# heracles-ec/heracles

Hardware: AMD Instinct MI355X
Metric: map->Cl pairs/sec + mixing-matrix build sec, nside=4096 lmax=6144 (higher is better)
Workload: dtype f64

## Files before the change

heracles_amd/_lib.py:

```python

from __future__ import annotations

import ctypes as C
import os
import threading

import numpy as np

_HERE = os.path.dirname(os.path.abspath(__file__))
_LIBNAME = os.environ.get("HX_LIBRARY") or os.path.join(_HERE, "libhxsht.so")
_lock = threading.Lock()
_lib = None

HX_OK = 0
HX_ERR_ARG, HX_ERR_NO_DEVICE, HX_ERR_HIP, HX_ERR_MEM, HX_ERR_UNSUPPORTED = -1, -2, -3, -4, -5

SYMBOLS = (
    "hx_version", "hx_last_error", "hx_device_count", "hx_init", "hx_set_stream",
    "hx_get_stream", "hx_set_async", "hx_synchronize", "hx_timer_start", "hx_timer_stop",
    "hx_profile_enable", "hx_profile_reset", "hx_profile_get", "hx_plan_create", "hx_set_max_lds_fft",
    "hx_plan_destroy", "hx_plan_scratch_bytes", "hx_plan_release_scratch", "hx_set_scratch_budget", "hx_plan_last_chunks", "hx_plan_mfma_flops", "hx_plan_executed_flops", "hx_executed_flops", "hx_measure_peaks", "hx_measured_mfma_clock", "hx_map2alm", "hx_map2alm_multi", "hx_map2alm_list", "hx_alm2map", "hx_copy",
    "hx_alm2cl_pairs", "hx_alm2cl_pairs_range", "hx_gauss_legendre", "hx_gauss_legendre_dd", "hx_wigner_d_table", "hx_mixmat",
    "hx_mixmat_eb", "hx_mixmat_eb_spin", "hx_mixmat_batch", "hx_mixctx_create", "hx_mixctx_apply", "hx_mixctx_apply_spin", "hx_mixctx_destroy", "hx_mixctx_set_bins", "hx_mixctx_apply_binned", "hx_mixctx_apply_binned_spin", "hx_cl2corr", "hx_corr2cl", "hx_cl2corr_cols", "hx_corr2cl_cols", "hx_cl2corr_cols_spin", "hx_corr2cl_cols_spin", "hx_xi_ratio", "hx_ang2pix_ring", "hx_map_values", "hx_ud_grade", "hx_reorder", "hx_matvec", "hx_pinv", "hx_alm_resample", "hx_region_maps", "hx_alm_subtract", "hx_fits_unpack_f64", "hx_fits_pack_f64", "hx_fits_unpack_columns",
    "hx_pointsht_create", "hx_pointsht_destroy", "hx_pointsht_info", "hx_pointsht_adjoint",
    "hx_pointsht_synthesis", "hx_pointsht_grids", "hx_pointgrid_gather", "hx_pointgrid_destroy",
    "hx_pixel_weights_size", "hx_pixel_weights_expand", "hx_pixel_weights_solve",
    "hx_ring_modes_size", "hx_ring_modes", "hx_legendre_from_modes", "hx_allgather_alms", "hx_host_alloc", "hx_host_free", "hx_mixmat_gemm_clock", "hx_mixmat_release", "hx_release_caches",
    "hx_cov_gram", "hx_cov_delete2", "hx_cov_shrink_sums",
    "hx_catmap_create", "hx_catmap_page", "hx_catmap_moments", "hx_catmap_finish", "hx_catmap_destroy",
    "hx_catalm_create", "hx_catalm_page", "hx_catalm_moments", "hx_catalm_finish", "hx_catalm_destroy",
    "hx_catmap_create_sel", "hx_catmap_page_sel", "hx_catmap_moments_sel", "hx_catmap_finish_sel", "hx_catmap_destroy_sel",
)


class HxError(RuntimeError):

    def __init__(self, code, msg):
        super().__init__(f"libhxsht error {code}: {msg}")
        self.code = code


def library_path() -> str:
    return _LIBNAME


def load():
    global _lib
    with _lock:
        if _lib is not None:
            return _lib
        if not os.path.exists(_LIBNAME):
            raise HxError(
                HX_ERR_NO_DEVICE,
                f"{_LIBNAME} not found: build it with `make -C heracles_amd/csrc` "
                "(hipcc, gfx950).  heracles_amd has no CPU fallback.",
            )
        try:
            import torch
        except ImportError:
            pass
        L = C.CDLL(_LIBNAME)
        vp, i, dp = C.c_void_p, C.c_int, C.c_void_p
        L.hx_version.restype = C.c_char_p
        L.hx_last_error.restype = C.c_char_p
        L.hx_get_stream.restype = vp
        L.hx_set_stream.argtypes = [vp]
        L.hx_plan_create.restype = vp
        L.hx_plan_create.argtypes = [i, i, i]
        L.hx_plan_destroy.argtypes = [vp]
        L.hx_plan_destroy.restype = None
        L.hx_plan_scratch_bytes.argtypes = [vp]
        L.hx_plan_scratch_bytes.restype = C.c_int64
        L.hx_plan_release_scratch.argtypes = [vp]
        L.hx_set_scratch_budget.argtypes = [C.c_double]
        L.hx_plan_last_chunks.argtypes = [vp]
        L.hx_plan_mfma_flops.argtypes = [vp, i, i, C.POINTER(C.c_double)]
        L.hx_plan_executed_flops.argtypes = [vp, i, i, C.POINTER(C.c_double)]
        L.hx_executed_flops.argtypes = [C.POINTER(C.c_double), i]
        L.hx_measure_peaks.argtypes = [C.POINTER(C.c_double)]
        L.hx_measured_mfma_clock.restype = C.c_double
        L.hx_map2alm.argtypes = [vp, i, i, dp, dp, dp, dp, dp, i]
        L.hx_alm2map.argtypes = [vp, i, i, dp, dp]
        L.hx_map2alm_multi.argtypes = [vp, i, vp, vp, vp, vp, dp, dp, vp]
        L.hx_map2alm_list.argtypes = [vp, i, vp, vp, vp, dp, dp, dp, dp, i]
        L.hx_copy.argtypes = [vp, vp, C.c_int64]
        L.hx_alm2cl_pairs.argtypes = [i, vp, vp, i, i, vp, vp, dp]
        L.hx_alm2cl_pairs_range.argtypes = [i, vp, vp, i, i, vp, vp, i, i, i, dp]
        L.hx_gauss_legendre.argtypes = [i, dp, dp]
        L.hx_gauss_legendre_dd.argtypes = [i, dp, dp, dp]
        L.hx_wigner_d_table.argtypes = [i, i, i, i, dp, dp]
        L.hx_mixmat.argtypes = [dp, i, i, i, i, i, i, dp]
        L.hx_mixmat_eb.argtypes = [dp, i, i, i, i, dp]
        L.hx_mixmat_eb_spin.argtypes = [dp, i, i, i, i, i, i, dp]
        L.hx_mixmat_batch.argtypes = [i, dp, i, i, i, i, vp, vp, vp, vp]
        L.hx_mixctx_create.restype = vp
        L.hx_mixctx_create.argtypes = [i, i, i]
        L.hx_mixctx_apply.argtypes = [vp, dp, i, i, dp]
        L.hx_mixctx_destroy.argtypes = [vp]
        L.hx_mixctx_set_bins.argtypes = [vp, i, vp, dp, dp]
        L.hx_mixctx_apply_binned.argtypes = [vp, dp, i, i, dp]
        L.hx_mixctx_apply_spin.argtypes = [vp, dp, i, i, i, dp]
        L.hx_mixctx_apply_binned_spin.argtypes = [vp, dp, i, i, i, dp]
        L.hx_mixctx_destroy.restype = None
        L.hx_cl2corr.argtypes = [i, i, dp, dp]
        L.hx_corr2cl.argtypes = [i, i, dp, dp]
        L.hx_cl2corr_cols.argtypes = [i, i, i, vp, dp, dp]
        L.hx_corr2cl_cols.argtypes = [i, i, i, vp, dp, dp]
        L.hx_cl2corr_cols_spin.argtypes = [i, i, i, vp, dp, dp]
        L.hx_corr2cl_cols_spin.argtypes = [i, i, i, vp, dp, dp]
        L.hx_xi_ratio.argtypes = [i, i, dp, dp, vp, dp, vp, vp, C.c_double, C.c_double, dp]
        L.hx_ang2pix_ring.argtypes = [i, C.c_int64, dp, dp, dp]
        L.hx_map_values.argtypes = [i, C.c_int64, dp, dp, i, dp, dp, i]
        L.hx_ud_grade.argtypes = [i, i, i, dp, dp]
        L.hx_reorder.argtypes = [i, i, i, dp, dp]
        L.hx_matvec.argtypes = [i, i, dp, i, dp, dp]
        L.hx_pinv.argtypes = [i, i, dp, C.c_double, dp, C.POINTER(C.c_double)]
        L.hx_alm_resample.argtypes = [i, i, i, dp, dp]
        L.hx_region_maps.argtypes = [C.c_int64, i, dp, dp, C.c_double, dp]
        L.hx_alm_subtract.argtypes = [C.c_int64, dp, i, vp, dp]
        L.hx_fits_unpack_f64.argtypes = [C.c_int64, i, i, C.c_int64, C.c_int64, C.c_int64, dp, dp]
        L.hx_fits_pack_f64.argtypes = [C.c_int64, i, i, C.c_int64, C.c_int64, C.c_int64, dp, dp]
        L.hx_fits_unpack_columns.argtypes = [C.c_int64, C.c_int64, i, vp, C.c_char_p, vp, vp, dp, vp, i]
        L.hx_pointsht_create.argtypes = [i, C.c_double]
        L.hx_pointsht_create.restype = vp
        L.hx_pointsht_destroy.argtypes = [vp]
        L.hx_pointsht_destroy.restype = None
        L.hx_pointsht_info.argtypes = [vp, C.POINTER(C.c_int)]
        L.hx_pointsht_adjoint.argtypes = [vp, i, i, C.c_int64, dp, dp, dp]
        L.hx_pointsht_synthesis.argtypes = [vp, i, i, C.c_int64, dp, dp, dp]
        L.hx_pointsht_grids.argtypes = [vp, i, i, dp]
        L.hx_pointsht_grids.restype = vp
        L.hx_pointgrid_gather.argtypes = [vp, C.c_int64, dp, dp]
        L.hx_pointgrid_destroy.argtypes = [vp]
        L.hx_pointgrid_destroy.restype = None
        L.hx_ring_modes_size.argtypes = [vp, i]
        L.hx_ring_modes_size.restype = C.c_int64
        L.hx_ring_modes.argtypes = [vp, i, dp, dp, dp, i, vp, vp, i, vp]
        L.hx_legendre_from_modes.argtypes = [vp, i, i, vp, i, i, i, dp, dp]
        L.hx_allgather_alms.argtypes = [vp, i, vp, dp]
        L.hx_pixel_weights_size.argtypes = [i]
        L.hx_pixel_weights_size.restype = C.c_int64
        L.hx_pixel_weights_expand.argtypes = [i, C.c_int64, dp, dp]
        L.hx_pixel_weights_solve.argtypes = [vp, i, C.c_double, i, dp, C.POINTER(C.c_int), C.POINTER(C.c_double), C.POINTER(C.c_double)]
        L.hx_host_alloc.argtypes = [C.c_int64, C.POINTER(C.c_void_p)]
        L.hx_host_free.argtypes = [vp]
        L.hx_mixmat_gemm_clock.restype = C.c_double
        L.hx_timer_stop.argtypes = [C.POINTER(C.c_float)]
        L.hx_cov_gram.argtypes = [i, i, i, dp, dp, C.c_double, dp]
        L.hx_cov_delete2.argtypes = [i, i, i, dp, dp, dp, vp, vp, i, vp, C.c_double, dp]
        L.hx_cov_shrink_sums.argtypes = [i, i, dp, dp, C.c_int64, dp]
        L.hx_catmap_create.restype = vp
        L.hx_catmap_create.argtypes = [C.c_int64, i, i, vp, vp]
        L.hx_catmap_page.argtypes = [vp, C.c_int64, vp]
        L.hx_catmap_moments.argtypes = [vp, dp, dp]
        L.hx_catmap_finish.argtypes = [vp, i, C.c_double, dp]
        L.hx_catmap_destroy.argtypes = [vp]
        L.hx_catmap_destroy.restype = None
        L.hx_catalm_create.restype = vp
        L.hx_catalm_create.argtypes = [C.c_int64, i, i, vp, vp]
        L.hx_catalm_page.argtypes = [vp, C.c_int64, vp]
        L.hx_catalm_moments.argtypes = [vp, dp, dp]
        L.hx_catalm_finish.argtypes = [vp, i, i, C.c_double, dp, dp]
        L.hx_catalm_destroy.argtypes = [vp]
        L.hx_catalm_destroy.restype = None
        L.hx_catmap_create_sel.restype = vp
        L.hx_catmap_create_sel.argtypes = [C.c_int64, i, i, vp, i, i, vp, vp, i, vp, vp, vp]
        L.hx_catmap_page_sel.argtypes = [vp, C.c_int64, vp, vp]
        L.hx_catmap_moments_sel.argtypes = [vp, dp, dp, dp]
        L.hx_catmap_finish_sel.argtypes = [vp, i, i, C.c_double, dp]
        L.hx_catmap_destroy_sel.argtypes = [vp]
        L.hx_catmap_destroy_sel.restype = None
        L.hx_profile_get.argtypes = [C.c_char_p, C.POINTER(C.c_int), C.POINTER(C.c_double)]
        _lib = L
        return L


def check(rc: int):
    if rc != HX_OK:
        raise HxError(rc, load().hx_last_error().decode(errors="replace"))


def ptr(obj):
    if obj is None:
        return None
    if isinstance(obj, int):
        return C.c_void_p(obj)
    if isinstance(obj, np.ndarray):
        if not obj.flags.c_contiguous:
            raise ValueError("array must be C-contiguous")
        return C.c_void_p(obj.ctypes.data)
    if hasattr(obj, "data_ptr"):
        if not obj.is_contiguous():
            raise ValueError("tensor must be contiguous")
        if getattr(obj, "is_cuda", False):
            import torch

            torch.cuda.current_stream(obj.device).synchronize()
        return C.c_void_p(obj.data_ptr())
    raise TypeError(f"cannot take the address of {type(obj)!r}")


def init(device: int | None = None):
    L = load()
    if device is None:
        device = int(os.environ.get("LOCAL_RANK", "0")) % max(L.hx_device_count(), 1)
    check(L.hx_init(int(device)))
    global _inited, _device
    _inited, _device = True, int(device)


_inited = False
_device = None


def ensure_init():
    global _inited
    if not _inited:
        init(None)
        _inited = True


def device() -> int:
    ensure_init()
    return _device


def device_count() -> int:
    return load().hx_device_count()


def measure_peaks():
    ensure_init()
    out = (C.c_double * 4)()
    check(load().hx_measure_peaks(out))
    return {"hbm_read_gbs": out[0], "hbm_copy_gbs": out[1], "fp64_mfma_tflops": out[2], "fp64_valu_tflops": out[3],
            "fp64_mfma_clock_ghz": load().hx_measured_mfma_clock()}


def synchronize():
    check(load().hx_synchronize())


def release_caches():
    from . import weights

    weights.release_computed()
    check(load().hx_release_caches())


def copy(dst, src):
    nb = int(src.nbytes) if hasattr(src, "nbytes") else int(src.numel() * src.element_size())
    nd = int(dst.nbytes) if hasattr(dst, "nbytes") else int(dst.numel() * dst.element_size())
    if nb != nd:
        raise ValueError(f"copy of {nb} bytes into {nd}")
    check(load().hx_copy(ptr(dst), ptr(src), nb))


def executed_flops(reset=False):
    ensure_init()
    out = (C.c_double * 2)()
    check(load().hx_executed_flops(out, 1 if reset else 0))
    return out[0], out[1]


def set_scratch_budget(nbytes: float):
    check(load().hx_set_scratch_budget(float(nbytes)))


class Timer:

    def __enter__(self):
        check(load().hx_timer_start())
        self.ms = None
        return self

    def __exit__(self, *exc):
        t = C.c_float()
        check(load().hx_timer_stop(C.byref(t)))
        self.ms = float(t.value)
        return False


def profile_enable(on=True):
    check(load().hx_profile_enable(1 if on else 0))


def profile_reset():
    check(load().hx_profile_reset())


def profile_get(name: str):
    n = C.c_int()
    ms = C.c_double()
    check(load().hx_profile_get(name.encode(), C.byref(n), C.byref(ms)))
    return n.value, ms.value


def pinned_empty(shape, dtype=None):
    import weakref

    dtype = np.dtype(np.float64 if dtype is None else dtype)
    shape = tuple(int(x) for x in (shape if isinstance(shape, (tuple, list)) else (shape,)))
    nbytes = int(np.prod(shape, dtype=np.int64)) * dtype.itemsize
    if nbytes == 0:
        return np.empty(shape, dtype)
    ensure_init()
    L = load()
    p = C.c_void_p()
    check(L.hx_host_alloc(C.c_int64(nbytes), C.byref(p)))
    raw = (C.c_char * nbytes).from_address(p.value)
    weakref.finalize(raw, L.hx_host_free, C.c_void_p(p.value))
    return np.frombuffer(raw, dtype=dtype).reshape(shape)


def result_array(shape, out=None):
    shape = tuple(int(x) for x in shape)
    if out is None:
        return np.empty(shape)
    if tuple(out.shape) != shape:
        raise ValueError(f"out has shape {tuple(out.shape)}, the result has {shape}")
    if isinstance(out, np.ndarray):
        if out.dtype != np.float64 or not out.flags.c_contiguous or not out.flags.writeable:
            raise ValueError("out must be a writeable C-contiguous float64 array")
    elif hasattr(out, "data_ptr"):
        import torch

        if out.dtype != torch.float64 or not out.is_contiguous():
            raise ValueError("out must be a contiguous float64 tensor")
    else:
        raise TypeError(f"out: cannot write into {type(out)!r}")
    return out
```

heracles_amd/csrc/hx_analysis.hip:

```cpp
#include <algorithm>
#include <cmath>
#include <cstdlib>
#include <cstring>

#include "hx_sht_common.h"

namespace hx {
using namespace hxfft;

constexpr int HALF_F = 1;
template <int SPIN>
struct LegCfg {
    static constexpr int NW = SPIN == 0 ? 16 : 8;
    static constexpr int NT = SPIN == 0 ? 1 : 2;
    static constexpr int NOP = SPIN == 0 ? 1 : 2;
    static constexpr int NPAR = (SPIN == 2 && HALF_F) ? 1 : 2;
};
int analysis_f_rows(int spin) { return spin == 0 ? LegCfg<0>::NPAR * LegCfg<0>::NOP : LegCfg<2>::NPAR * LegCfg<2>::NOP; }

struct LegParams {
    PlanDev P;
    const LegTask *__restrict__ tasks;
    const double *__restrict__ F;
    double *__restrict__ partial;
    int m0, ms;
    long long row0;
    int ng;
    int ncol;
    int pcol;
    const MTasks *__restrict__ of_m;
    const long long *__restrict__ arow;
    long long arow0;
    int add_all;
};

constexpr int COMB_NXCD = 8, COMB_XG = 4;
constexpr int COMB_TM = 16;
constexpr int COMB_IPT = 3;
constexpr int COMB_MPAD = 2;
static int combine_rp(int rowlen) { return rowlen <= 40 ? 8 : 4; }
static size_t combine_lds_bytes(int rp, int rowlen)
{
    return (size_t)COMB_TM * ((size_t)rp * rowlen + COMB_MPAD) * sizeof(double) + (size_t)COMB_TM * rp * sizeof(RingAtM) + COMB_TM * sizeof(int);
}
template <int SPIN, int RP>
__global__ __launch_bounds__(1024) void k_fourier_combine(PlanDev P, const double2 *__restrict__ Y, int ncomp, int ncol, int m0, int ms,
                                                         int nm, int kshift, int gx, int gy, const double *__restrict__ rw,
                                                         const LegTask *__restrict__ tasks, const MTasks *__restrict__ of_m,
                                                         double *__restrict__ F, int tile0)
{
    constexpr int NOP = LegCfg<SPIN>::NOP, NPAR = LegCfg<SPIN>::NPAR, TM = COMB_TM;
    const int bq = (int)blockIdx.x / (COMB_NXCD * COMB_XG), br = (int)blockIdx.x % (COMB_NXCD * COMB_XG);
    const int t = (bq * COMB_NXCD + br % COMB_NXCD) * COMB_XG + br / COMB_NXCD;
    if (t >= gx * gy) return;
    const int tx = t % gx, ty = t / gx;
    static_assert(TM == 16 && 32 % RP == 0 && TM * RP <= 256, "tile shape");
    extern __shared__ __align__(16) unsigned char comb_lds[];
    const int rowlen = NPAR * NOP * ncol;
    const int mstride = RP * rowlen + COMB_MPAD;
    double *tile = reinterpret_cast<double *>(comb_lds);
    RingAtM *ring_at_m = reinterpret_cast<RingAtM *>(tile + TM * mstride);
    int *m_live = reinterpret_cast<int *>(ring_at_m + TM * RP);
    const int kb = tx * TM - kshift;
    const int rp0 = (ty + tile0 * (32 / RP)) * RP;
    if (threadIdx.x < TM * RP) {
        const int mi = threadIdx.x % TM, j = threadIdx.x / TM, k = kb + mi;
        bool on = k >= 0 && k < nm;
        if (on) {
            const int m = m0 + k * ms;
            const MTasks mt = of_m[m];
            on = mt.count != 0 && rp0 / 32 >= tasks[mt.first].rb0;
            if (on) ring_at_m[j * TM + mi] = ring_at_m_of(P, rp0 + j, m, rw);
        }
        if (j == 0) m_live[mi] = on;
    }
    __syncthreads();
    const int nsl = ncol >> 1;
    for (int e = threadIdx.x; e < RP * nsl * TM; e += blockDim.x) {
        const int i = e % TM, sj = e / TM, s = sj % nsl, j = sj / nsl;
        const int mi = ((i & 3) << 2) | (i >> 2);
        if (!m_live[mi]) continue;
        const int m = m0 + (kb + mi) * ms, rp = rp0 + j;
        const bool live = rp < P.nrp;
        const RingAtM ram = ring_at_m[j * TM + mi];
        double *row = tile + mi * mstride + j * rowlen;
        if (SPIN == 0) {
            const int c = s;
            double2 sm = make_double2(0.0, 0.0), d = sm;
            if (live && c < ncomp) {
                double2 fn, fs;
                ring_modes_ns(P, Y, c, rp, m, ram, fn, fs);
                sm = cadd(fn, fs);
                d = csub(fn, fs);
            }
            *reinterpret_cast<double2 *>(row + 2 * s) = sm;
            *reinterpret_cast<double2 *>(row + ncol + 2 * s) = d;
        } else {
            const int f = s >> 1, op = s & 1;
            double4 o0 = make_double4(0.0, 0.0, 0.0, 0.0), o1 = o0;
            if (live && 2 * f + 1 < ncomp) {
                double2 qn, qs, un, us;
                ring_modes_ns(P, Y, 2 * f, rp, m, ram, qn, qs);
                ring_modes_ns(P, Y, 2 * f + 1, rp, m, ram, un, us);
                const double2 ppn = cscale(cadd(qn, mul_pi(un)), -0.5), pmn = cscale(csub(qn, mul_pi(un)), -0.5);
                const double2 pps = cscale(cadd(qs, mul_pi(us)), -0.5), pms = cscale(csub(qs, mul_pi(us)), -0.5);
                double4 x, y;
                if (op == 0) {
                    x = make_double4(ppn.x, ppn.y, ppn.y, -ppn.x);
                    y = make_double4(pms.x, pms.y, -pms.y, pms.x);
                } else {
                    x = make_double4(pmn.x, pmn.y, -pmn.y, pmn.x);
                    y = make_double4(pps.x, pps.y, pps.y, -pps.x);
                }
                o0 = make_double4(x.x + y.x, x.y + y.y, x.z + y.z, x.w + y.w);
                o1 = make_double4(x.x - y.x, x.y - y.y, x.z - y.z, x.w - y.w);
            }
            double2 *t0 = reinterpret_cast<double2 *>(row + (0 * NOP + op) * ncol + 4 * f);
            t0[0] = make_double2(o0.x, o0.y);
            t0[1] = make_double2(o0.z, o0.w);
            if (NPAR == 2) {
                double2 *t1 = reinterpret_cast<double2 *>(row + (1 * NOP + op) * ncol + 4 * f);
                t1[0] = make_double2(o1.x, o1.y);
                t1[1] = make_double2(o1.z, o1.w);
            }
        }
    }
    __syncthreads();
    const int lane = threadIdx.x & 63, npiece = RP * rowlen / 2, cpm = (npiece + 63) / 64;
    for (int ch = threadIdx.x >> 6; ch < TM * cpm; ch += blockDim.x >> 6) {
        const int mi = ch / cpm, u = (ch % cpm) * 64 + lane;
        if (!m_live[mi] || u >= npiece) continue;
        const double2 *src = reinterpret_cast<const double2 *>(tile + mi * mstride);
        double2 *dst = reinterpret_cast<double2 *>(F + ((long long)(kb + mi) * P.nrp_pad + rp0) * rowlen);
        dst[u] = src[u];
    }
}

template <int SPIN>
static void launch_fourier_combine(hipStream_t st, const PlanDev &P, const double2 *Y, int ncomp, int ncol, int m0, int ms, int nm, const double *d_rw,
                                   const LegTask *tasks, const MTasks *of_m, double *F, int tile0, int ntile32)
{
    const int kshift = ms == 1 ? m0 % COMB_TM : 0;
    const int rowlen = LegCfg<SPIN>::NPAR * LegCfg<SPIN>::NOP * ncol;
    const int gx = (nm + kshift + COMB_TM - 1) / COMB_TM;
    static_assert((size_t)COMB_TM * (4 * LegCfg<SPIN>::NPAR * LegCfg<SPIN>::NOP * (NCOL * NGMAX + 8) + COMB_MPAD) * sizeof(double) +
                          (size_t)COMB_TM * 4 * sizeof(RingAtM) + COMB_TM * sizeof(int) <= 65536, "a tile of 4 ring pairs must fit 64 KiB of LDS");
    const int rp = combine_rp(rowlen), items = rp * (ncol / 2) * COMB_TM;
    const unsigned nt = (unsigned)std::min(1024, std::max(COMB_TM * rp, (items / COMB_IPT + 63) / 64 * 64));
    const int gy = ntile32 * (32 / rp);
    const dim3 grid((unsigned)((gx * gy + COMB_NXCD * COMB_XG - 1) / (COMB_NXCD * COMB_XG) * (COMB_NXCD * COMB_XG)));
    const size_t lds = combine_lds_bytes(rp, rowlen);
    if (rp == 8)
        hipLaunchKernelGGL((k_fourier_combine<SPIN, 8>), grid, dim3(nt), lds, st, P, Y, ncomp, ncol, m0, ms, nm, kshift, gx, gy, d_rw, tasks, of_m, F, tile0);
    else
        hipLaunchKernelGGL((k_fourier_combine<SPIN, 4>), grid, dim3(nt), lds, st, P, Y, ncomp, ncol, m0, ms, nm, kshift, gx, gy, d_rw, tasks, of_m, F, tile0);
}

__device__ __host__ inline int tile_swz(int r) { return r & 15; }
__device__ __host__ inline int ringsel(int q, int k) { return (k & 1) * 16 + 2 * q + (k >> 1); }

template <int K>
__device__ inline int opaque(int v)
{
    asm("; opaque %1" : "+v"(v) : "n"(K));
    return v;
}

__device__ unsigned long long g_exec_flops[2];

template <int SPIN>
struct PipeCfg {
    static constexpr int NW = 4;
    static constexpr int RBS = SPIN == 0 ? 2 : 1;
    static constexpr int NCH = SPIN == 0 ? 2 : 1;
    static constexpr int NOP = SPIN == 0 ? 1 : 2;
};

__device__ __host__ inline int pipe_rho(int q, int k) { return 4 * q + k; }
__device__ __host__ inline int pipe_tile_idx(int c, int r) { return c * 32 + ((r ^ (c & 7)) * 2); }

constexpr int DUO_GAP = -1;
constexpr int DUO_PRIO = 1;
constexpr int DUO_ORDER = -1;
constexpr int DUO_SCALE_BITS2 = 100;
constexpr int DUO_SCALE_BITS0 = 300;

template <int K>
__device__ __forceinline__ double row_bcast(double v)
{
    double d;
    asm("v_mov_b64_dpp %0, %1 row_newbcast:%2 row_mask:0xf bank_mask:0xf" : "=v"(d) : "v"(v), "n"(K));
    return d;
}

template <int K>
__device__ __forceinline__ double row_bcast_fmac(double t, double p, double x)
{
    asm("v_fmac_f64_dpp %0, %1, %2 row_newbcast:%3 row_mask:0xf bank_mask:0xf" : "+v"(t) : "v"(p), "v"(x), "n"(K));
    return t;
}

template <int SPIN>
__device__ __forceinline__ void alm_rows_to_layout(const PlanDev &P, int m, bool any_task, const double *__restrict__ partial, long long r0, int ncol,
                                                   int ncomp, int ng, const double *__restrict__ fl, int add, double2 *__restrict__ alm,
                                                   long long alm_stride, const double *__restrict__ alphan, int tid, int nt)
{
    const int lmax = P.lmax;
    const int l0 = SPIN == 0 ? m : (m > 2 ? m : 2);
    const int nl = lmax - m + 1, nc = 8 * ng;
    constexpr int U = 8;
    for (int i0 = tid; i0 < nl * nc; i0 += nt * U) {
        double2 v[U];
        double al[U], f[U];
        long long dsti[U];
        bool on[U];
#pragma unroll
        for (int u = 0; u < U; ++u) {
            const int i = i0 + u * nt;
            const int l = m + i / nc, c = i % nc;
            on[u] = i < nl * nc && c < ncomp;
            v[u] = make_double2(0.0, 0.0);
            al[u] = 1.0;
            f[u] = 1.0;
            dsti[u] = 0;
            if (!on[u]) continue;
            dsti[u] = (long long)c * alm_stride + almidx(lmax, l, m);
            if (l >= l0 && any_task) {
                const double *prow = partial + (r0 + (l - l0)) * ncol + (c >> 3) * NCOL;
                v[u] = *reinterpret_cast<const double2 *>(prow + 2 * (c & 7));
                if (SPIN == 2 && alphan && ((l + m) & 1)) {
                    const int j = 2 * (c & 7);
                    v[u] = make_double2(prow[j ^ 3], prow[(j + 1) ^ 3]);
                }
                if (SPIN == 2 && HALF_F && ((l + m) & 1)) {
                    if (c & 1) v[u].y = -v[u].y;
                    else v[u].x = -v[u].x;
                }
                if (alphan) al[u] = alphan[almidx(lmax, l, m)];
                if (fl) f[u] = fl[l];
            }
        }
#pragma unroll
        for (int u = 0; u < U; ++u) {
            if (!on[u]) continue;
            double2 w = v[u];
            if (alphan) { w.x *= al[u]; w.y *= al[u]; }
            if (fl) { w.x *= f[u]; w.y *= f[u]; }
            double2 *dst = alm + dsti[u];
            if (add) { const double2 o = *dst; w.x += o.x; w.y += o.y; }
            *dst = w;
        }
    }
}

template <int SPIN, int NG, int NBX, int NSUB = 1>
__global__ __launch_bounds__(256, 2) void k_legendre_duo(LegParams A, const double2 *__restrict__ coefn)
{
    using C = PipeCfg<SPIN>;
    constexpr int NW = 4, NOP = C::NOP, NCH = C::NCH, NPAIR = 16;
    constexpr int NXA = NBX > 0 ? NBX : 1;
    constexpr int DQ0 = NG * 512, DSZ = NG * 512 + NBX * 128;
    constexpr bool HALFB = SPIN == 2;
    constexpr int SB = SPIN == 2 ? DUO_SCALE_BITS2 : DUO_SCALE_BITS0;
    constexpr int GAPN = DUO_GAP >= 0 ? DUO_GAP : ((SPIN == 2 && NG == 2 && NBX == 2) ? 5 : (SPIN == 2 && NG == 2 && NBX == 1) ? 6 : (SPIN == 2 && NG == 1 && NBX == 2) ? 0 : 4);
    constexpr int GORDER = DUO_ORDER >= 0 ? DUO_ORDER : ((SPIN == 2 && NG == 2 && NBX == 2) ? 2 : (SPIN == 0 && NG == 1 && NBX == 1) ? 1 : 0);
    constexpr int NPB = HALFB ? 1 : 2;
    constexpr int TW = NSUB * DSZ > 2048 ? NSUB * DSZ : 2048;
    static_assert(NG >= 1 && NG <= 2 && TW * NW * 8 <= 81920, "two work-groups per CU");
    static_assert(SPIN == 0 || HALF_F, "spin 2: the lambda- chain carries (-1)^(l + m) lambda- (one operand row, wave-uniform coefficients)");
    __shared__ double tile[NW][TW];
    __shared__ int lead_in[2][NW];
    const PlanDev &P = A.P;
    const int m = A.m0 + blockIdx.x * A.ms, lmax = P.lmax;
    const MTasks mt = A.of_m[m];
    const int l0 = SPIN == 0 ? m : (m > 2 ? m : 2);
    const int off = (l0 + m) & 1;
    const int nblk = (lmax - l0) / LBLK + 1;
    const long long orow = A.arow[m] - A.arow0;
    const double2 *__restrict__ cfm = coefn + almidx(lmax, 0, m) + l0 + (SPIN == 0 ? 0 : 1) + (threadIdx.x & 15);
    bool first_group = true;
    auto put = [&](double *p, double v) __attribute__((always_inline)) {
        if (first_group) *p = v;
        else __builtin_amdgcn_global_atomic_fadd_f64((__attribute__((address_space(1))) double *)p, v);
    };
    auto lds_barrier = []() __attribute__((always_inline)) {
        __builtin_amdgcn_s_waitcnt(0xc07f);
        __builtin_amdgcn_s_barrier();
    };
    int n_mf = 0, n_rec = 0;
    if (DUO_PRIO) __builtin_amdgcn_s_setprio(3);
    for (int ti = 0; ti < mt.count; ++ti) {
        const LegTask task = A.tasks[mt.first + ti];
        first_group = ti == 0 && !A.add_all;
        int tid = threadIdx.x;
        asm volatile("; ring group" : "+v"(tid));
        const int w = tid >> 6, lane = tid & 63;
        const int ai = lane & 15, ak = lane >> 4;
        if (ti) __syncthreads();

        const int rbi = SPIN == 0 ? 2 * w + (lane >> 5) : w;
        const int rpl = (task.rb0 + rbi) * RBLK + (lane & 31);
        const bool valid = rbi < task.nrb && rpl < P.nrp;
        const double x = valid ? P.z[rpl] : 0.0;
        const double xx = SPIN == 0 ? x * x : ((lane >> 5) ? -x : x);

        double fr[NPAIR][NPB][NG], frx[NPAIR][NPB][NXA];
#pragma unroll
        for (int sp = 0; sp < NPAIR; ++sp) {
            const int op = SPIN == 0 ? 0 : sp & 1, q = SPIN == 0 ? sp : sp >> 1;
            const int rbq = SPIN == 0 ? 2 * w + (q >> 3) : w;
            const bool on = rbq < task.nrb;
            const long long row = (long long)blockIdx.x * P.nrp_pad + (task.rb0 + rbq) * RBLK + pipe_rho(q & 7, ak);
            if (HALFB) {
                const double *f = A.F + (row * NOP + op) * A.ncol;
#pragma unroll
                for (int g = 0; g < NG; ++g) fr[sp][0][g] = on ? f[g * NCOL + ai] : 0.0;
#pragma unroll
                for (int g = 0; g < NXA; ++g) frx[sp][0][g] = (NBX > 0 && on) ? f[NG * NCOL + 4 * g + (lane & 3)] : 0.0;
            } else {
#pragma unroll
                for (int pos = 0; pos < NPB; ++pos) {
                    const double *f = A.F + ((row * 2 + (pos ^ off)) * NOP + op) * A.ncol;
#pragma unroll
                    for (int g = 0; g < NG; ++g) fr[sp][pos][g] = on ? f[g * NCOL + ai] : 0.0;
#pragma unroll
                    for (int g = 0; g < NXA; ++g) frx[sp][pos][g] = (NBX > 0 && on) ? f[NG * NCOL + 4 * g + (lane & 3)] : 0.0;
                }
            }
        }

        double vc[NCH], vp[NCH];
        int sc[NCH];
#pragma unroll
        for (int c = 0; c < NCH; ++c) { vc[c] = 0.0; vp[c] = 0.0; sc[c] = -100; }
        if (valid) {
            if (SPIN == 0) {
                SVal a = spow(P.sth[rpl], m);
                a.v *= P.mfac[m];
                SVal b = a;
                b.v *= sqrt(2.0 * m + 3.0) * P.z[rpl];
                snorm_small(a);
                snorm_small(b);
                vc[0] = a.v; sc[0] = a.e;
                vc[NCH - 1] = b.v; sc[NCH - 1] = b.e;
            } else {
                SVal sp, sm;
                spin2_seeds(m, P.sth[rpl], P.omz[rpl], P.kfac2[m], sp, sm);
                vc[0] = (lane >> 5) ? (off ? -sm.v : sm.v) : sp.v;
                sc[0] = (lane >> 5) ? sm.e : sp.e;
            }
#pragma unroll
            for (int c = 0; c < NCH; ++c) sval_rebase<SB>(vc[c], sc[c]);
        }

        auto rec_step = [&](auto RMM, int c, int step, const double tq) __attribute__((always_inline)) {
            constexpr int RM = decltype(RMM)::value;
            if (RM != 3 && (step & 3) == 0) {
                const int hc = __double2hiint(vc[c]), hp = __double2hiint(vp[c]);
                const bool up = sc[c] < 0 && (hc & 0x7ff00000) >= 0x3ff00000;
                const int sub = up ? (SB << 20) : 0;
                const bool pz = up && (hp & 0x7ff00000) <= (SB << 20);
                vc[c] = __hiloint2double(hc - sub, __double2loint(vc[c]));
                vp[c] = pz ? 0.0 : __hiloint2double(hp - sub, __double2loint(vp[c]));
                sc[c] += up ? 1 : 0;
            }
            const double cur = (RM == 3 || sc[c] == 0) ? vc[c] : 0.0;
            const double vn = fma(tq, vc[c], -vp[c]);
            vp[c] = vc[c];
            vc[c] = vn;
            return cur;
        };
        constexpr int HB = 8;
        double *tw = &tile[w][0];
        auto recursion = [&](auto RMM, const double2 (&cl)[2]) __attribute__((always_inline)) {
            constexpr int RM = decltype(RMM)::value;
#pragma unroll
            for (int h = 0; h < LBLK / HB; ++h) {
                double cur[HB];
#pragma unroll
                for (int k = 0; k < HB; ++k) {
                    constexpr int dummy = 0; (void)dummy;
                    const int kk = HB * h + k;
                    double tq = 0.0;
                    switch (kk & 15) {
#define HX_BC(K) case K: tq = row_bcast_fmac<K>(row_bcast<K>(cl[kk >> 4].y), cl[kk >> 4].x, xx); break;
                        HX_BC(0) HX_BC(1) HX_BC(2) HX_BC(3) HX_BC(4) HX_BC(5) HX_BC(6) HX_BC(7)
                        HX_BC(8) HX_BC(9) HX_BC(10) HX_BC(11) HX_BC(12) HX_BC(13) HX_BC(14) HX_BC(15)
#undef HX_BC
                    }
                    cur[k] = rec_step(RMM, SPIN == 0 ? ((kk & 1) ? NCH - 1 : 0) : 0, SPIN == 0 ? kk >> 1 : kk, tq);
                }
                if (RM >= 2) {
#pragma unroll
                    for (int j = 0; j < HB / 2; ++j)
                        *reinterpret_cast<double2 *>(tw + pipe_tile_idx(lane, h * (HB / 2) + j)) = make_double2(cur[2 * j], cur[2 * j + 1]);
                }
                __builtin_amdgcn_sched_barrier(0);
            }
        };
        auto set_mode = [&](int b) __attribute__((always_inline)) {
            const int eb = b == 0 ? 60 : (b == 1 ? 34 : (30 - 2 * b > 8 ? 30 - 2 * b : 8));
            auto lane_dead = [&](int c) __attribute__((always_inline)) {
                if (SB == 300) return sc[c] < 0;
                const int ef = (__double2hiint(vc[c]) >> 20) & 0x7ff;
                return sc[c] <= -2 || (sc[c] == -1 && ef <= 1022 - eb);
            };
            bool dead = !valid || lane_dead(0), live = !valid || sc[0] == 0;
            if (NCH == 2) {
                dead = dead && (!valid || lane_dead(NCH - 1));
                live = live && (!valid || sc[NCH - 1] == 0);
            }
            return __all(dead) ? 1 : (__all(live) ? 3 : 2);
        };
        using I1 = std::integral_constant<int, 1>;
        using I2 = std::integral_constant<int, 2>;
        using I3 = std::integral_constant<int, 3>;

        const int fcol = tid & 15, fch = (tid >> 4) & 7, fpos = (tid >> 7) & 1;
        const int frow = (fch >> 1) + 8 * (fch & 1);
        const int qrow = tid / (4 * NXA), qcol = tid % (4 * NXA);
        double *pgrp = A.partial + (orow + 2 * frow + fpos) * A.pcol + fcol;
        double *pquad = A.partial + (orow + 2 * qrow) * A.pcol + NG * NCOL + qcol;
        double2 cnext[2] = {cfm[0], cfm[16]};
        bool started = first_group;
        int nflush = 0;
        for (int b0 = 0; b0 < nblk; b0 += NSUB) {
            double4_t acc[NSUB][NG][2];
            double accx[NSUB][NXA][2];
            bool mine = false;
#pragma unroll
            for (int sub = 0; sub < NSUB; ++sub) {
                const int b = b0 + sub;
#pragma unroll
                for (int g = 0; g < NG; ++g) acc[sub][g][0] = acc[sub][g][1] = (double4_t){0.0, 0.0, 0.0, 0.0};
#pragma unroll
                for (int g = 0; g < NXA; ++g) accx[sub][g][0] = accx[sub][g][1] = 0.0;
                if (b >= nblk) break;
                int rm = set_mode(b);
                const double2 cl[2] = {cnext[0], cnext[1]};
                if (rm == 3) recursion(I3{}, cl);
                else if (rm == 2) {
                    recursion(I2{}, cl);
                    if (SB != 300) {
                        bool lv = valid && sc[0] == 0;
                        if (NCH == 2) lv = lv || (valid && sc[NCH - 1] == 0);
                        if (!__any(lv)) rm = 1;
                    }
                } else recursion(I1{}, cl);
                cnext[0] = cfm[(b + 1) * LBLK];
                cnext[1] = cfm[(b + 1) * LBLK + 16];
                n_rec = __builtin_amdgcn_readfirstlane(n_rec + 1);
                mine = mine || rm >= 2;
                if (rm >= 2) {
                    n_mf = __builtin_amdgcn_readfirstlane(n_mf + 1);
                    if (DUO_PRIO) __builtin_amdgcn_s_setprio(0);
                    constexpr int PF = 3;
                    auto a_fetch = [&](int sp) __attribute__((always_inline)) {
                        const int op = SPIN == 0 ? 0 : sp & 1, q = SPIN == 0 ? sp : sp >> 1;
                        const int c = SPIN == 0 ? (q >> 3) * 32 + pipe_rho(q & 7, ak) : op * 32 + pipe_rho(q, ak);
                        return *reinterpret_cast<const double2 *>(tw + pipe_tile_idx(c, ai));
                    };
                    double2 aq[PF + 1];
#pragma unroll
                    for (int j = 0; j < PF; ++j) aq[j] = a_fetch(j);
#pragma unroll
                    for (int sp = 0; sp < NPAIR; ++sp) {
                        if (sp + PF < NPAIR) aq[(sp + PF) % (PF + 1)] = a_fetch(sp + PF);
                        const double a0 = aq[sp % (PF + 1)].x, a1 = aq[sp % (PF + 1)].y;
#pragma unroll
                        for (int pos = 0; pos < 2; ++pos) {
                            const double a = pos ? a1 : a0;
                            if (GAPN > 0) {
                                if (GORDER == 1) {
#pragma unroll
                                for (int g = 0; g < (NG > NBX ? NG : NBX); ++g) {
                                    if (g < NG) acc[sub][g][pos] = __builtin_amdgcn_mfma_f64_16x16x4f64(a, fr[sp][HALFB ? 0 : pos][g], acc[sub][g][pos], 0, 0, 0);
                                    __builtin_amdgcn_sched_barrier(0);
                                    asm volatile("s_nop %0" ::"n"(GAPN > 0 ? GAPN - 1 : 0));
                                    __builtin_amdgcn_sched_barrier(0);
                                    if (g < NBX) accx[sub][g][pos] = __builtin_amdgcn_mfma_f64_4x4x4f64(a, frx[sp][HALFB ? 0 : pos][g], accx[sub][g][pos], 0, 0, 0);
                                    __builtin_amdgcn_sched_barrier(0);
                                }
                                } else if (GORDER == 2) {
#pragma unroll
                                for (int g = 0; g < NG; ++g) acc[sub][g][pos] = __builtin_amdgcn_mfma_f64_16x16x4f64(a, fr[sp][HALFB ? 0 : pos][g], acc[sub][g][pos], 0, 0, 0);
                                __builtin_amdgcn_sched_barrier(0);
                                asm volatile("s_nop %0" ::"n"(GAPN > 0 ? GAPN - 1 : 0));
                                __builtin_amdgcn_sched_barrier(0);
#pragma unroll
                                for (int g = 0; g < NBX; ++g) accx[sub][g][pos] = __builtin_amdgcn_mfma_f64_4x4x4f64(a, frx[sp][HALFB ? 0 : pos][g], accx[sub][g][pos], 0, 0, 0);
                                __builtin_amdgcn_sched_barrier(0);
                                if (NBX > 0) asm volatile("s_nop %0" ::"n"(GAPN > 0 ? GAPN - 1 : 0));
                                __builtin_amdgcn_sched_barrier(0);
                                } else {
#pragma unroll
                                for (int g = 0; g < (NG > NBX ? NG : NBX); ++g) {
                                    if (g < NG) acc[sub][g][pos] = __builtin_amdgcn_mfma_f64_16x16x4f64(a, fr[sp][HALFB ? 0 : pos][g], acc[sub][g][pos], 0, 0, 0);
                                    if (g < NBX) accx[sub][g][pos] = __builtin_amdgcn_mfma_f64_4x4x4f64(a, frx[sp][HALFB ? 0 : pos][g], accx[sub][g][pos], 0, 0, 0);
                                    __builtin_amdgcn_sched_barrier(0);
                                    asm volatile("s_nop %0" ::"n"(GAPN > 0 ? GAPN - 1 : 0));
                                    __builtin_amdgcn_sched_barrier(0);
                                }
                                }
                            } else {
#pragma unroll
                                for (int g = 0; g < NG; ++g) acc[sub][g][pos] = __builtin_amdgcn_mfma_f64_16x16x4f64(a, fr[sp][HALFB ? 0 : pos][g], acc[sub][g][pos], 0, 0, 0);
#pragma unroll
                                for (int g = 0; g < NBX; ++g) accx[sub][g][pos] = __builtin_amdgcn_mfma_f64_4x4x4f64(a, frx[sp][HALFB ? 0 : pos][g], accx[sub][g][pos], 0, 0, 0);
                            }
                        }
                        __builtin_amdgcn_sched_barrier(0);
                    }
                    if (DUO_PRIO) __builtin_amdgcn_s_setprio(3);
                }
            }
            const bool two = NSUB > 1 && b0 + 1 < nblk;
            if (!started) {
                if (lane == 0) lead_in[nflush & 1][w] = mine ? 1 : 0;
                lds_barrier();
                const int4 fl = *reinterpret_cast<const int4 *>(&lead_in[nflush & 1][0]);
                ++nflush;
                started = __builtin_amdgcn_readfirstlane(fl.x | fl.y | fl.z | fl.w) != 0;
                if (!started) {
                    pgrp += (long long)NSUB * LBLK * A.pcol;
                    pquad += (long long)NSUB * LBLK * A.pcol;
                    continue;
                }
            }
#pragma unroll
            for (int sub = 0; sub < NSUB; ++sub) {
                double *dt = tw + sub * DSZ;
#pragma unroll
                for (int g = 0; g < NG; ++g)
#pragma unroll
                    for (int pos = 0; pos < 2; ++pos)
#pragma unroll
                        for (int h = 0; h < 2; ++h)
                            *reinterpret_cast<double2 *>(dt + (g * 2 + pos) * 256 + ai * 16 + (((2 * ak + h) ^ (ai & 7)) * 2)) = make_double2(acc[sub][g][pos][2 * h], acc[sub][g][pos][2 * h + 1]);
#pragma unroll
                for (int g = 0; g < NBX; ++g)
                    *reinterpret_cast<double2 *>(dt + DQ0 + ((4 * ((lane >> 2) & 3) + ak) * 4 * NBX + 4 * g + (lane & 3)) * 2) = make_double2(accx[sub][g][0], accx[sub][g][1]);
            }
            lds_barrier();
#pragma unroll
            for (int sub = 0; sub < NSUB; ++sub) {
                if (sub > 0 && !two) break;
                const long long rsub = (long long)sub * LBLK * A.pcol;
#pragma unroll
                for (int g = 0; g < NG; ++g) {
                    const double *src = &tile[0][0] + sub * DSZ + (g * 2 + fpos) * 256 + fcol * 16 + ((fch ^ (fcol & 7)) * 2);
                    double2 s4[NW];
#pragma unroll
                    for (int ww = 0; ww < NW; ++ww) s4[ww] = *reinterpret_cast<const double2 *>(src + ww * TW);
                    put(pgrp + rsub + g * NCOL, (s4[0].x + s4[1].x) + (s4[2].x + s4[3].x));
                    put(pgrp + rsub + g * NCOL + 8 * (long long)A.pcol, (s4[0].y + s4[1].y) + (s4[2].y + s4[3].y));
                }
                if (NBX > 0 && tid < 64 * NBX) {
                    double2 s4[NW];
#pragma unroll
                    for (int ww = 0; ww < NW; ++ww) s4[ww] = *reinterpret_cast<const double2 *>(&tile[0][0] + ww * TW + sub * DSZ + DQ0 + tid * 2);
                    put(pquad + rsub, (s4[0].x + s4[1].x) + (s4[2].x + s4[3].x));
                    put(pquad + rsub + A.pcol, (s4[0].y + s4[1].y) + (s4[2].y + s4[3].y));
                }
            }
            pgrp += (long long)NSUB * LBLK * A.pcol;
            pquad += (long long)NSUB * LBLK * A.pcol;
            lds_barrier();
        }
    }
    if ((threadIdx.x & 63) == 0) {
        atomicAdd(&g_exec_flops[0], (unsigned long long)n_mf * (32ull * (NG * 2048ull + NBX * 512ull)));
        atomicAdd(&g_exec_flops[1], (unsigned long long)n_rec * (64ull * LBLK * 4ull));
    }
}

template <int SPIN>
__global__ __launch_bounds__(256) void k_alm_reduce(PlanDev P, const LegTask *__restrict__ tasks,
                                                    const MTasks *__restrict__ of_m,
                                                    const double *__restrict__ partial, long long row0, int m0, int ms,
                                                    int ncomp, int ng, int ncol, const double *__restrict__ fl, int add,
                                                    double2 *__restrict__ alm, long long alm_stride,
                                                    const long long *__restrict__ arow, const double *__restrict__ alphan)
{
    const int m = m0 + blockIdx.x * ms, lmax = P.lmax;
    const int l0 = SPIN == 0 ? m : (m > 2 ? m : 2);
    const MTasks mt = of_m[m];
    const int nl = lmax - m + 1, nc = 8 * ng;
    if (arow) {
        alm_rows_to_layout<SPIN>(P, m, mt.count > 0, partial, arow[m] - row0, ncol, ncomp, ng, fl, add, alm, alm_stride, alphan, threadIdx.x, blockDim.x);
        return;
    }
    for (int i = threadIdx.x; i < nl * nc; i += blockDim.x) {
        const int l = m + i / nc, c = i % nc;
        if (c >= ncomp) continue;
        double2 v = make_double2(0.0, 0.0);
        if (l >= l0) {
            const int col = (c >> 3) * NCOL + 2 * (c & 7);
            for (int t = 0; t < mt.count; ++t) {
                const double *p = partial + (tasks[mt.first + t].pout - row0 + (l - l0)) * ncol + col;
                v.x += p[0];
                v.y += p[1];
            }
            if (fl) { v.x *= fl[l]; v.y *= fl[l]; }
        }
        double2 *dst = alm + (long long)c * alm_stride + almidx(lmax, l, m);
        if (add) { const double2 o = *dst; v.x += o.x; v.y += o.y; }
        *dst = v;
    }
}

__global__ __launch_bounds__(256) void k_alm_reduce_spin(int lmax, int s, const LegTask *__restrict__ tasks, const MTasks *__restrict__ of_m,
                                                         const double *__restrict__ partial, long long row0, int m0, int ms,
                                                         const double *__restrict__ fl, int add, double2 *__restrict__ alm, long long alm_stride)
{
    const int m = m0 + blockIdx.x * ms;
    const int l0 = m > s ? m : s;
    const MTasks mt = of_m[m];
    const int nl = lmax - m + 1;
    for (int i = threadIdx.x; i < nl * 2; i += blockDim.x) {
        const int l = m + (i >> 1), c = i & 1;
        double2 v = make_double2(0.0, 0.0);
        if (l >= l0) {
            for (int t = 0; t < mt.count; ++t) {
                const double *p = partial + (tasks[mt.first + t].pout - row0 + (l - l0)) * 4 + 2 * c;
                v.x += p[0];
                v.y += p[1];
            }
            if (fl) { v.x *= fl[l]; v.y *= fl[l]; }
        }
        double2 *dst = alm + (long long)c * alm_stride + almidx(lmax, l, m);
        if (add) { const double2 o = *dst; v.x += o.x; v.y += o.y; }
        *dst = v;
    }
}

struct SweepShape {
    int ng, nbx, valu, ncol, duo;
};
static SweepShape sweep_shape(int spin, int nb)
{
    const int cols = 2 * nb;
    SweepShape sh = {0, 0, 0, 0, 0};
    if (cols <= 8) { sh.valu = 1; return sh; }
    sh.duo = 1;
    sh.ng = std::max(cols / NCOL, 1);
    const int rem = cols > NCOL ? cols % NCOL : 0;
    const int maxbx = spin == 2 ? 2 : (sh.ng == 1 ? 1 : 0);
    if (rem > 4 * maxbx) sh.ng += 1;
    else sh.nbx = (rem + 3) / 4;
    sh.ncol = NCOL * sh.ng + 4 * sh.nbx;
    return sh;
}
bool analysis_generic_spin(int spin)
{
    if (spin != 2) return spin != 0;
    const char *e = getenv("HX_SPIN_GENERIC");
    return e && atoi(e) != 0;
}
int analysis_max_comp(int spin) { return spin == 2 ? 8 * NGMAX + 4 : 8 * NGMAX; }

static double sweep_cost(int spin, int units)
{
    if (spin == 0) return units <= 4 ? 21.6 * units : (units <= 8 ? 84.1 : (units <= 10 ? 99.2 : 139.7));
    return units <= 2 ? 61.0 * units : (units <= 4 ? 164.5 : (units == 5 ? 194.1 : (units == 6 ? 222.0 : (units <= 8 ? 272.0 : (units == 9 ? 299.6 : 326.0)))));
}
int analysis_next_batch(int spin, int remaining)
{
    const int unit = spin == 0 ? 1 : 2, maxu = analysis_max_comp(spin) / unit;
    const int units = remaining / unit;
    if (units <= 0) return 0;
    std::vector<double> best(units + 1, 0.0);
    std::vector<int> first(units + 1, 0);
    for (int r = 1; r <= units; ++r) {
        best[r] = 1e300;
        for (int b = std::min(maxu, r); b >= 1; --b) {
            const double c = sweep_cost(spin, b) + best[r - b];
            if (c < best[r] - 1e-9) { best[r] = c; first[r] = b; }
        }
    }
    return unit * first[units];
}
int analysis_max_batch(int spin, int ncomp)
{
    int mx = 0;
    for (int left = ncomp; left > 0;) {
        const int nb = analysis_next_batch(spin, left);
        if (nb <= 0) break;
        mx = std::max(mx, nb);
        left -= nb;
    }
    return mx;
}

int one_set_task_blocks(int spin) { return PipeCfg<2>::NW * (spin ? PipeCfg<2>::RBS : PipeCfg<0>::RBS); }
int flop_task_blocks(int spin) { return spin == 0 ? LegCfg<0>::NW : LegCfg<2>::NW; }

static bool duo_shape(const SweepShape &sh) { return sh.duo != 0; }
static int sweep_pcol(const SweepShape &sh) { return sh.ncol > 2 * NCOL ? (sh.ncol + 15) / 16 * 16 : sh.ncol; }

template <int SPIN>
static int launch_duo(const SweepShape &sh, dim3 pgrid, hipStream_t st, const LegParams &A, const double2 *cn)
{
    const dim3 db(256);
    const int key = sh.ng * 10 + sh.nbx;
    if (key == 10) hipLaunchKernelGGL((k_legendre_duo<SPIN, 1, 0, 2>), pgrid, db, 0, st, A, cn);
    else if (key == 11) hipLaunchKernelGGL((k_legendre_duo<SPIN, 1, 1, 2>), pgrid, db, 0, st, A, cn);
    else if (key == 20 && SPIN == 2) hipLaunchKernelGGL((k_legendre_duo<2, 2, 0, 2>), pgrid, db, 0, st, A, cn);
    else if (key == 12 && SPIN == 2) hipLaunchKernelGGL((k_legendre_duo<2, 1, 2, 2>), pgrid, db, 0, st, A, cn);
    else if (key == 21 && SPIN == 2) hipLaunchKernelGGL((k_legendre_duo<2, 2, 1, 2>), pgrid, db, 0, st, A, cn);
    else if (key == 20) hipLaunchKernelGGL((k_legendre_duo<SPIN, 2, 0>), pgrid, db, 0, st, A, cn);
    else if (key == 22 && SPIN == 2) hipLaunchKernelGGL((k_legendre_duo<2, 2, 2>), pgrid, db, 0, st, A, cn);
    else return fail(HX_ERR_ARG, "legendre analysis: no two-group kernel for %d groups + %d blocks", sh.ng, sh.nbx);
    return HX_OK;
}

static void launch_alm_reduce(hx_plan *pl, int spin, hx_plan::TaskSet &ts, long long row0, int m0, int ms, int nm, int nb, int ng, int pcol,
                              const double *d_fl, int add, double2 *d_alms, const double *al)
{
    const PlanDev P = pl->dev();
    const long long *arow = al ? ts.d_arow.as<long long>() : nullptr;
    if (spin == 0)
        hipLaunchKernelGGL(k_alm_reduce<0>, dim3(nm), dim3(256), 0, rt().stream, P, ts.d_tasks.as<LegTask>(), ts.d_of_m.as<MTasks>(), pl->partial.as<double>(),
                           row0, m0, ms, nb, ng, pcol, d_fl, add, d_alms, pl->nlm, arow, al);
    else
        hipLaunchKernelGGL(k_alm_reduce<2>, dim3(nm), dim3(256), 0, rt().stream, P, ts.d_tasks.as<LegTask>(), ts.d_of_m.as<MTasks>(), pl->partial.as<double>(),
                           row0, m0, ms, nb, ng, pcol, d_fl, add, d_alms, pl->nlm, arow, al);
}

template <int SPIN>
static int launch_chunk(hx_plan *pl, hx_plan::SpinData &sd, hx_plan::TaskSet &ts, int m0, int m1, int nb, const SweepShape &sh, const double *d_rw,
                        const double *d_fl, int add, double2 *d_alms)
{
    const int ng = sh.ng + (sh.nbx > 0 ? 1 : 0), ncol = sh.ncol;
    const int pcol = sweep_pcol(sh);
    hipStream_t st = rt().stream;
    PlanDev P = pl->dev();
    const int t0 = ts.of_m[m0].first;
    const int t1 = ts.of_m[m1 - 1].first + ts.of_m[m1 - 1].count;
    const int ms = std::max(pl->m_step, 1), nm = (m1 - m0 + ms - 1) / ms;
    {
        ProfScope ps("fourier_combine");
        launch_fourier_combine<SPIN>(st, P, pl->Y.as<double2>(), nb, ncol, m0, ms, nm, d_rw, ts.d_tasks.as<LegTask>(), ts.d_of_m.as<MTasks>(),
                                     pl->F.as<double>(), 0, pl->nrp_pad / 32);
    }
    if (t1 > t0) {
        ProfScope ps("legendre_analysis");
        ProfScope ps2(SPIN == 0 ? "legendre_analysis_s0" : "legendre_analysis_s2");
        LegParams A;
        A.P = P; A.tasks = ts.d_tasks.as<LegTask>() + t0; A.F = pl->F.as<double>(); A.partial = pl->partial.as<double>();
        A.m0 = m0; A.ms = ms; A.row0 = ts.rows_before_m[m0]; A.ng = ng; A.ncol = ncol; A.pcol = pcol;
        A.of_m = ts.d_of_m.as<MTasks>(); A.arow = ts.d_arow.as<long long>(); A.arow0 = ts.arow[m0]; A.add_all = 0;
        A.tasks = ts.d_tasks.as<LegTask>();
        HX_TRY(launch_duo<SPIN>(sh, dim3((unsigned)nm), st, A, sd.cn.as<double2>()));
    }
    {
        ProfScope ps("alm_reduce");
        launch_alm_reduce(pl, SPIN, ts, ts.arow[m0], m0, ms, nm, nb, ng, pcol, d_fl, add, d_alms, sd.al.as<double>());
    }
    HX_HIP(hipGetLastError());
    return HX_OK;
}

static bool valu_batch(int spin, int nb) { return sweep_shape(spin, nb).valu != 0; }

static double analysis_budget(const hx_plan *pl)
{
    if (scratch_budget_bytes() > 0.0) return scratch_budget_bytes();
    double budget = 80e9;
    size_t fr = 0, tot = 0;
    if (hipMemGetInfo(&fr, &tot) == hipSuccess) budget = std::min(budget, 0.5 * (double)(fr + pl->F.bytes + pl->partial.bytes));
    return std::max(budget, 2e9);
}

static int plan_m_chunks(hx_plan *pl, double f_per_m, const std::vector<long long> &prow, size_t row_bytes, std::vector<std::pair<int, int>> &chunks)
{
    const double budget = analysis_budget(pl);
    size_t maxF = 16, maxP = 16;
    const int m_end = pl->m_hi < 0 ? pl->lmax + 1 : std::min(pl->m_hi, pl->lmax + 1), ms = std::max(pl->m_step, 1);
    for (int m0 = std::max(pl->m_lo, 0); m0 < m_end;) {
        int last = m0;
        while (last + ms < m_end) {
            const double bytes = f_per_m * ((last + ms - m0) / ms + 1) + (double)(prow[last + ms + 1] - prow[m0]) * row_bytes;
            if (bytes > budget) break;
            last += ms;
        }
        const int m1 = last + 1;
        chunks.emplace_back(m0, m1);
        maxF = std::max(maxF, (size_t)(f_per_m * ((m1 - m0 + ms - 1) / ms)));
        maxP = std::max(maxP, (size_t)(prow[m1] - prow[m0]) * row_bytes);
        m0 = last + ms;
    }
    HX_TRY(pl->F.alloc(maxF));
    HX_TRY(pl->partial.alloc(maxP));
    pl->last_chunks = (int)chunks.size();
    return HX_OK;
}

static int analysis_batch_valu(hx_plan *pl, int spin, int nb, const double *d_maps, double2 *d_alms, const double *d_rw,
                               const double *d_pw, const double *d_fl, int add, bool generic = false)
{
    hx_plan::SpinData *sd = nullptr;
    hx_plan::TaskSet *tsp = nullptr;
    HX_TRY(spin_data(pl, spin, generic, &sd));
    HX_TRY(task_set(pl, spin, generic, valu_task_blocks(spin), &tsp));
    hx_plan::TaskSet &ts = *tsp;
    if (pl->hsrc == nullptr && pl->nssrc == nullptr) {
        HX_TRY(pl->Y.alloc(sizeof(double2) * (size_t)pl->ny * nb));
        HX_TRY(launch_ring_subdft_maps(pl, nb, d_maps, d_pw, pl->Y.as<double2>()));
    }
    const int lmax = pl->lmax, pcol = valu_partial_cols(spin), unit = spin ? 2 : 1, ms = std::max(pl->m_step, 1);
    std::vector<std::pair<int, int>> chunks;
    HX_TRY(plan_m_chunks(pl, (double)pl->nrp_pad * valu_operand_doubles(spin) * sizeof(double), ts.rows_before_m, pcol * sizeof(double), chunks));
    for (int c0 = 0; c0 < nb; c0 += unit)
        for (auto &ch : chunks) {
            const int m0 = ch.first, m1 = ch.second, nm = (m1 - m0 + ms - 1) / ms;
            HX_TRY(launch_valu_chunk(pl, spin, *sd, ts, m0, m1, c0, d_rw, generic));
            ProfScope ps("alm_reduce");
            if (generic)
                hipLaunchKernelGGL(k_alm_reduce_spin, dim3(nm), dim3(256), 0, rt().stream, lmax, spin, ts.d_tasks.as<LegTask>(), ts.d_of_m.as<MTasks>(),
                                   pl->partial.as<double>(), ts.rows_before_m[m0], m0, ms, d_fl, add, d_alms + (size_t)c0 * pl->nlm, pl->nlm);
            else
                launch_alm_reduce(pl, spin, ts, ts.rows_before_m[m0], m0, ms, nm, unit, 1, pcol, d_fl, add, d_alms + (size_t)c0 * pl->nlm, nullptr);
            HX_HIP(hipGetLastError());
        }
    return HX_OK;
}

int analysis_batch(hx_plan *pl, int spin, int nb, const double *d_maps, double2 *d_alms, const double *d_rw,
                   const double *d_pw, const double *d_fl, int add)
{
    const bool generic = plan_generic_spin(pl, spin);
    if (generic || (spin != 0 && spin != 2)) {
        if (!generic) return fail(HX_ERR_UNSUPPORTED, "spin-%d maps not yet supported", spin);
        if (spin < 0 || nb < 2 || (nb & 1)) return fail(HX_ERR_ARG, "analysis_batch: %d components of spin %d", nb, spin);
        if (spin > pl->lmax) {
            if (!add) HX_HIP(hipMemsetAsync(d_alms, 0, sizeof(double2) * (size_t)pl->nlm * nb, rt().stream));
            return HX_OK;
        }
        return analysis_batch_valu(pl, spin, nb, d_maps, d_alms, d_rw, d_pw, d_fl, add, true);
    }
    if (valu_batch(spin, nb)) return analysis_batch_valu(pl, spin, nb, d_maps, d_alms, d_rw, d_pw, d_fl, add);
    const SweepShape sh = sweep_shape(spin, nb);
    hx_plan::TaskSet *ts = nullptr;
    hx_plan::SpinData *sd = nullptr;
    HX_TRY(spin_data(pl, spin, false, &sd));
    HX_TRY(task_set(pl, spin, false, one_set_task_blocks(spin), &ts));
    if (pl->hsrc == nullptr && pl->nssrc == nullptr) {
        HX_TRY(pl->Y.alloc(sizeof(double2) * (size_t)pl->ny * nb));
        HX_TRY(launch_ring_subdft_maps(pl, nb, d_maps, d_pw, pl->Y.as<double2>()));
    }
    std::vector<std::pair<int, int>> chunks;
    HX_TRY(plan_m_chunks(pl, (double)pl->nrp_pad * analysis_f_rows(spin) * sh.ncol * sizeof(double), ts->arow, sweep_pcol(sh) * sizeof(double), chunks));
    for (auto &ch : chunks) {
        if (spin == 0)
            HX_TRY(launch_chunk<0>(pl, *sd, *ts, ch.first, ch.second, nb, sh, d_rw, d_fl, add, d_alms));
        else
            HX_TRY(launch_chunk<2>(pl, *sd, *ts, ch.first, ch.second, nb, sh, d_rw, d_fl, add, d_alms));
    }
    return HX_OK;
}

bool analysis_can_stream(hx_plan *pl, int spin, int nb)
{
    if (!pl || pl->nside < 1 || pl->hsrc || pl->nssrc || pl->m_lo != 0 || pl->m_hi >= 0 || pl->m_step > 1) return false;
    if (nb < 1 || nb > analysis_max_comp(spin)) return false;
    const SweepShape sh = sweep_shape(spin, nb);
    if (!duo_shape(sh) || sh.valu) return false;
    const double f_bytes = (double)pl->nrp_pad * analysis_f_rows(spin) * sh.ncol * sizeof(double) * (pl->lmax + 1.0);
    const double p_bytes = 0.5 * (pl->lmax + 1.0) * (pl->lmax + 2.0 + LBLK) * sweep_pcol(sh) * sizeof(double);
    double budget = 80e9;
    if (scratch_budget_bytes() > 0.0) budget = scratch_budget_bytes();
    if (f_bytes + p_bytes > budget) return false;
    size_t fr = 0, tot = 0;
    if (hipMemGetInfo(&fr, &tot) != hipSuccess) {
        (void)hipGetLastError();
        return false;
    }
    const double y_bytes = (double)pl->ny * nb * sizeof(double2), stage_bytes = 2.0 * nb * (double)pl->npix * sizeof(double);
    const double held = (double)pl->F.bytes + (double)pl->partial.bytes + (double)pl->Y.bytes + (double)pl->stage[0].bytes + (double)pl->stage[1].bytes +
                        (double)pl->stage[2].bytes;
    return f_bytes + p_bytes + y_bytes + stage_bytes <= 0.95 * ((double)fr + held);
}

int analysis_stream_plan(hx_plan *pl, int spin, int nb, int nslab, StreamSweep &s)
{
    if (!analysis_can_stream(pl, spin, nb)) return fail(HX_ERR_ARG, "analysis_stream_plan: not a streamable sweep");
    HX_TRY(spin_data(pl, spin, false, &s.sd));
    HX_TRY(task_set(pl, spin, false, one_set_task_blocks(spin), &s.ts));
    hx_plan::TaskSet &ts = *s.ts;
    const SweepShape sh = sweep_shape(spin, nb);
    s.pl = pl; s.spin = spin; s.nb = nb;
    const int nrb = (pl->nrp + RBLK - 1) / RBLK;
    std::vector<double> cum(nrb + 1, 0.0);
    for (int rb = 0; rb < nrb; ++rb) {
        double px = 0.0;
        for (int rp = rb * RBLK; rp < std::min((rb + 1) * RBLK, pl->nrp); ++rp) px += (rp == pl->nrp - 1 ? 4.0 : 8.0) * pl->h_nsub[rp];
        cum[rb + 1] = cum[rb] + px;
    }
    nslab = std::max(1, std::min(nslab, nrb));
    s.rp_edge.assign(1, 0);
    for (int k = 1; k < nslab; ++k) {
        const int rb = (int)(std::lower_bound(cum.begin(), cum.end(), cum[nrb] * k / nslab) - cum.begin());
        if (rb * RBLK > s.rp_edge.back() && rb < nrb) s.rp_edge.push_back(rb * RBLK);
    }
    s.rp_edge.push_back(nrb * RBLK);
    s.nslab = (int)s.rp_edge.size() - 1;
    const int lmax = pl->lmax;
    std::vector<MTasks> tab((size_t)s.nslab * (lmax + 1), MTasks{0, 0});
    for (int m = 0; m <= lmax; ++m) {
        const MTasks mt = ts.of_m[m];
        int t = mt.first;
        for (int k = 0; k < s.nslab; ++k) {
            const int rb_hi = s.rp_edge[k + 1] / RBLK;
            MTasks &o = tab[(size_t)k * (lmax + 1) + m];
            o.first = t;
            while (t < mt.first + mt.count && ts.tasks[t].rb0 + ts.tasks[t].nrb <= rb_hi) ++t;
            o.count = t - o.first;
        }
        if (t != mt.first + mt.count) return fail(HX_ERR_ARG, "analysis_stream_plan: ring groups of m = %d left over", m);
    }
    HX_TRY(upload(s.d_of_m, tab));
    HX_TRY(pl->Y.alloc(sizeof(double2) * (size_t)pl->ny * nb));
    HX_TRY(pl->F.alloc((size_t)pl->nrp_pad * analysis_f_rows(spin) * sh.ncol * sizeof(double) * (size_t)(lmax + 1)));
    HX_TRY(pl->partial.alloc((size_t)ts.arow[lmax + 1] * sweep_pcol(sh) * sizeof(double)));
    return HX_OK;
}

int analysis_stream_start(StreamSweep &s)
{
    hx_plan *pl = s.pl;
    const SweepShape sh = sweep_shape(s.spin, s.nb);
    HX_HIP(hipMemsetAsync(pl->partial.p, 0, (size_t)s.ts->arow[pl->lmax + 1] * sweep_pcol(sh) * sizeof(double), rt().stream));
    pl->last_chunks = 1;
    return HX_OK;
}

template <int SPIN>
static int stream_slab(StreamSweep &s, int k)
{
    hx_plan *pl = s.pl;
    hx_plan::TaskSet &ts = *s.ts;
    const SweepShape sh = sweep_shape(SPIN, s.nb);
    const int ng = sh.ng + (sh.nbx > 0 ? 1 : 0), lmax = pl->lmax, nm = lmax + 1;
    const int rp_lo = s.rp_edge[k], rp_hi = s.rp_edge[k + 1];
    hipStream_t st = rt().stream;
    PlanDev P = pl->dev();
    HX_TRY(launch_ring_subdft_maps(pl, s.nb, s.d_maps, s.d_pw, pl->Y.as<double2>(), rp_lo, std::min(rp_hi, pl->nrp)));
    {
        ProfScope ps("fourier_combine");
        const int tile_hi = k + 1 == s.nslab ? pl->nrp_pad / 32 : rp_hi / 32;
        launch_fourier_combine<SPIN>(st, P, pl->Y.as<double2>(), s.nb, sh.ncol, 0, 1, nm, s.d_rw, ts.d_tasks.as<LegTask>(), ts.d_of_m.as<MTasks>(),
                                     pl->F.as<double>(), rp_lo / 32, tile_hi - rp_lo / 32);
    }
    {
        ProfScope ps("legendre_analysis");
        ProfScope ps2(SPIN == 0 ? "legendre_analysis_s0" : "legendre_analysis_s2");
        LegParams A;
        A.P = P; A.tasks = ts.d_tasks.as<LegTask>(); A.F = pl->F.as<double>(); A.partial = pl->partial.as<double>();
        A.m0 = 0; A.ms = 1; A.row0 = 0; A.ng = ng; A.ncol = sh.ncol; A.pcol = sweep_pcol(sh);
        A.of_m = s.d_of_m.as<MTasks>() + (size_t)k * (lmax + 1); A.arow = ts.d_arow.as<long long>(); A.arow0 = 0; A.add_all = 1;
        HX_TRY(launch_duo<SPIN>(sh, dim3((unsigned)nm), st, A, s.sd->cn.as<double2>()));
    }
    HX_HIP(hipGetLastError());
    return HX_OK;
}

int analysis_stream_slab(StreamSweep &s, int k)
{
    if (k < 0 || k >= s.nslab) return fail(HX_ERR_ARG, "analysis_stream_slab: slab %d of %d", k, s.nslab);
    return s.spin == 0 ? stream_slab<0>(s, k) : stream_slab<2>(s, k);
}

int analysis_stream_end(StreamSweep &s)
{
    hx_plan *pl = s.pl;
    const SweepShape sh = sweep_shape(s.spin, s.nb);
    ProfScope ps("alm_reduce");
    launch_alm_reduce(pl, s.spin, *s.ts, 0LL, 0, 1, pl->lmax + 1, s.nb, sh.ng + (sh.nbx > 0 ? 1 : 0), sweep_pcol(sh), s.d_fl, 0, s.d_alms, s.sd->al.as<double>());
    HX_HIP(hipGetLastError());
    return HX_OK;
}

static int flop_wave_blocks(hx_plan *pl, int spin, double *out)
{
    hx_plan::TaskSet *ts = nullptr;
    HX_TRY(task_set(pl, spin, false, flop_task_blocks(spin), &ts));
    *out = 0.0;
    for (const LegTask &t : ts->tasks) *out += (double)t.nrb * ((pl->lmax - std::max(t.m, spin)) / LBLK + 1);
    return HX_OK;
}

}

extern "C" int hx_plan_mfma_flops(hx_plan *pl, int spin, int ncomp, double *flops)
{
    using namespace hx;
    if (!pl || !flops || ncomp < 1 || (spin != 0 && spin != 2)) return fail(HX_ERR_ARG, "hx_plan_mfma_flops: bad arguments");
    HX_TRY(ensure_ready());
    double wave_blocks = 0.0;
    HX_TRY(flop_wave_blocks(pl, spin, &wave_blocks));
    const int nop = spin ? 2 : 1;
    double per_wave_block = 0.0;
    for (int c0 = 0, nb = 0; c0 < ncomp; c0 += nb) {
        nb = analysis_next_batch(spin, ncomp - c0);
        const SweepShape sh = sweep_shape(spin, nb);
        per_wave_block += 16.0 * nop * (sh.ng * 2048.0 + sh.nbx * 512.0);
    }
    *flops = wave_blocks * per_wave_block;
    return HX_OK;
}

extern "C" int hx_executed_flops(double *out2, int reset)
{
    using namespace hx;
    if (!out2) return fail(HX_ERR_ARG, "hx_executed_flops: null output");
    HX_TRY(ensure_ready());
    HX_HIP(hipStreamSynchronize(rt().stream));
    unsigned long long v[2] = {0, 0}, w = 0;
    HX_HIP(hipMemcpyFromSymbol(v, HIP_SYMBOL(g_exec_flops), sizeof(v)));
    HX_TRY(valu_exec_flops(&w, reset != 0));
    if (reset) {
        const unsigned long long z[2] = {0, 0};
        HX_HIP(hipMemcpyToSymbol(HIP_SYMBOL(g_exec_flops), z, sizeof(z)));
    }
    out2[0] = (double)v[0];
    out2[1] = (double)v[1] + (double)w;
    return HX_OK;
}

extern "C" int hx_plan_executed_flops(hx_plan *pl, int spin, int ncomp, double *out2)
{
    using namespace hx;
    if (!out2) return fail(HX_ERR_ARG, "hx_plan_executed_flops: null output");
    HX_TRY(hx_plan_mfma_flops(pl, spin, ncomp, &out2[0]));
    double wave_blocks = 0.0;
    HX_TRY(flop_wave_blocks(pl, spin, &wave_blocks));
    const int nop = spin ? 2 : 1;
    int sweeps = 0;
    for (int c0 = 0, nb = 0; c0 < ncomp; c0 += nb, ++sweeps) nb = analysis_next_batch(spin, ncomp - c0);
    out2[1] = wave_blocks * sweeps * (double)RBLK * LBLK * nop * 4.0;
    return HX_OK;
}
```

heracles_amd/csrc/hx_map2alm.hip:

```cpp
#include <algorithm>
#include <chrono>
#include <cstdlib>

#include "hx_sht_common.h"
#include "hx_sweep_plan.h"

using namespace hx;

int hx::check_sht_args(hx_plan *pl, int spin, int ncomp, const void *a, const void *b, bool any_spin)
{
    if (!pl || !a || !b) return fail(HX_ERR_ARG, "null plan or buffer");
    if (pl->nside < 1) return fail(HX_ERR_ARG, "not a HEALPix plan");
    if (spin < 0 && any_spin) return fail(HX_ERR_ARG, "negative spin weight %d", spin);
    if (spin != 0 && spin != 2 && !any_spin) return fail(HX_ERR_UNSUPPORTED, "spin-%d maps not yet supported", spin);
    if (ncomp < 1 || (spin >= 1 && (ncomp & 1))) return fail(HX_ERR_ARG, "bad component count %d for spin %d", ncomp, spin);
    return HX_OK;
}

namespace hx {
__global__ void k_apply_fl(int lmax, int ncomp, long long nlm, const double *__restrict__ fl, double2 *__restrict__ alm)
{
    const int m = blockIdx.x;
    for (int i = threadIdx.x; i < (lmax - m + 1) * ncomp; i += blockDim.x) {
        const int c = i / (lmax - m + 1), l = m + i % (lmax - m + 1);
        double2 *p = alm + c * nlm + almidx(lmax, l, m);
        p->x *= fl[l];
        p->y *= fl[l];
    }
}
}

static int apply_fl(hx_plan *pl, int nb, double2 *alm, const double *fl)
{
    hipLaunchKernelGGL(k_apply_fl, dim3(pl->lmax + 1), dim3(256), 0, rt().stream, pl->lmax, nb, pl->nlm, fl, alm);
    HX_HIP(hipGetLastError());
    return HX_OK;
}

static int push(void *dst, const double *src, size_t bytes, hipStream_t on)
{
    if (is_device_ptr(src)) HX_HIP(hipMemcpyAsync(dst, src, bytes, hipMemcpyDeviceToDevice, on ? on : rt().stream));
    else HX_TRY(copy_h2d(dst, src, bytes, on));
    return HX_OK;
}

template <class Src>
static int gather_components(double *dst, int ncomp, long long npix, Src src, hipStream_t on)
{
    for (int c = 0, e; c < ncomp; c = e) {
        for (e = c + 1; e < ncomp && src(e) == src(e - 1) + npix; ++e) {}
        HX_TRY(push(dst + (size_t)c * npix, src(c), sizeof(double) * (size_t)(e - c) * npix, on));
    }
    return HX_OK;
}

static int map2alm_multi_impl(hx_plan *pl, int njobs, const int *spins, const int *ncomps, const double *const *maps, const double *const *const *comp_maps,
                              double *const *alms, const double *ring_weights, const double *pix_weights, const double *const *fls)
{
    HX_TRY(ensure_ready());
    if (!pl || njobs < 1 || !spins || !ncomps || !maps || !alms) return fail(HX_ERR_ARG, "hx_map2alm_multi: bad arguments");
    for (int j = 0; j < njobs; ++j) HX_TRY(check_sht_args(pl, spins[j], ncomps[j], maps[j], alms[j]));
    std::vector<bool> staged(njobs);
    InView vrw, vpw;
    HX_TRY(vrw.bind(ring_weights, sizeof(double) * pl->nrp));
    HX_TRY(vpw.bind(pix_weights, sizeof(double) * (size_t)pl->npix));
    HX_TRY(classify_pixel_weights(pl, vpw.as<double>()));
    std::vector<InView> vfl(njobs);
    std::vector<OutView> valm(njobs);
    static int want_slabs = -1;
    if (want_slabs < 0) { const char *e = getenv("HX_STREAM_SLABS"); want_slabs = e ? atoi(e) : 12; }
    bool any_host = false;
    for (int j = 0; j < njobs; ++j) {
        HX_TRY(vfl[j].bind(fls ? fls[j] : nullptr, sizeof(double) * (pl->lmax + 1)));
        HX_TRY(valm[j].bind(alms[j], sizeof(double2) * (size_t)ncomps[j] * pl->nlm));
        staged[j] = !is_device_ptr(maps[j]) || (comp_maps && comp_maps[j]);
        any_host = any_host || staged[j];
    }
    auto can_stream = [&](int spin, int nb) { return want_slabs > 1 && copy_stream() != nullptr && analysis_can_stream(pl, spin, nb); };
    std::vector<Sweep> sweeps = plan_sweeps(njobs, spins, ncomps, staged, analysis_next_batch, can_stream);
    hipStream_t cs = any_host ? copy_stream() : nullptr;
    size_t stage_bytes = 0;
    for (const Sweep &w : sweeps)
        if (staged[w.job]) stage_bytes = std::max(stage_bytes, (size_t)(sizeof(double) * (size_t)w.nb * (size_t)pl->npix));
    const int NST = 3 * (double)stage_bytes > 64e9 ? 2 : hx_plan::NSTAGE;
    constexpr int NEV = hx_plan::NUNIT_EV;
    hipEvent_t *unit_up = pl->unit_up;
    if (any_host) {
        if (!cs) return fail(HX_ERR_HIP, "hx_map2alm_multi: no copy stream");
        for (int i = 0; i < NST; ++i) {
            HX_TRY(pl->stage[i].alloc(stage_bytes));
            if (!pl->stage_done[i]) HX_HIP(hipEventCreateWithFlags(&pl->stage_done[i], hipEventDisableTiming));
        }
        for (int i = 0; i < NEV; ++i)
            if (!unit_up[i]) HX_HIP(hipEventCreateWithFlags(&unit_up[i], hipEventDisableTiming));
    }
    std::vector<int> hidx(sweeps.size(), -1);
    int nh = 0;
    for (size_t k = 0; k < sweeps.size(); ++k)
        if (staged[sweeps[k].job]) hidx[k] = nh++;
    std::vector<StreamSweep> ss(sweeps.size());
    for (size_t k = 0; k < sweeps.size(); ++k) {
        const Sweep &w = sweeps[k];
        if (!w.stream) continue;
        HX_TRY(analysis_stream_plan(pl, spins[w.job], w.nb, want_slabs, ss[k]));
        ss[k].d_maps = pl->stage[hidx[k] % NST].as<double>();
        ss[k].d_alms = valm[w.job].as<double2>() + (size_t)w.c0 * pl->nlm;
        ss[k].d_rw = vrw.as<double>(); ss[k].d_pw = vpw.as<double>(); ss[k].d_fl = vfl[w.job].as<double>();
    }
    struct Unit { size_t k; int slab; };
    std::vector<Unit> units;
    for (size_t k = 0; k < sweeps.size(); ++k) {
        if (sweeps[k].stream)
            for (int q = 0; q < ss[k].nslab; ++q) units.push_back({k, q});
        else
            units.push_back({k, -1});
    }
    std::vector<int> uidx(units.size(), -1);
    int nu = 0;
    for (size_t u = 0; u < units.size(); ++u)
        if (hidx[units[u].k] >= 0) uidx[u] = nu++;
    auto comp_src = [&](const Sweep &w, int c) -> const double * {
        return (comp_maps && comp_maps[w.job]) ? comp_maps[w.job][w.c0 + c] : maps[w.job] + (size_t)(w.c0 + c) * pl->npix;
    };
    auto upload = [&](size_t u) -> int {
        const Sweep &w = sweeps[units[u].k];
        const int b = hidx[units[u].k] % NST, slab = units[u].slab;
        if (slab <= 0 && hidx[units[u].k] >= NST) HX_HIP(hipEventSynchronize(pl->stage_done[b]));
        double *stage = pl->stage[b].as<double>();
        if (slab < 0) {
            HX_TRY(gather_components(stage, w.nb, pl->npix, [&](int c) { return comp_src(w, c); }, cs));
        } else {
            const StreamSweep &sw = ss[units[u].k];
            const int r0 = sw.rp_edge[slab], r1 = std::min(sw.rp_edge[slab + 1], pl->nrp) - 1;
            const long long n0 = pl->h_startN[r0], n1 = pl->h_startN[r1] + 4LL * pl->h_nsub[r1];
            const int rs = pl->h_startS[r1] >= 0 ? r1 : r1 - 1;
            const long long s0 = rs >= r0 ? pl->h_startS[rs] : 0, s1 = rs >= r0 ? pl->h_startS[r0] + 4LL * pl->h_nsub[r0] : 0;
            for (int c = 0; c < w.nb; ++c) {
                const double *src = comp_src(w, c);
                double *dst = stage + (size_t)c * pl->npix;
                HX_TRY(push(dst + n0, src + n0, sizeof(double) * (size_t)(n1 - n0), cs));
                if (s1 > s0) HX_TRY(push(dst + s0, src + s0, sizeof(double) * (size_t)(s1 - s0), cs));
            }
        }
        HX_HIP(hipEventRecord(unit_up[uidx[u] % NEV], cs));
        return HX_OK;
    };
    auto next_upload = [&](size_t u) -> size_t {
        for (size_t q = u + 1; q < units.size(); ++q)
            if (uidx[q] >= 0) return q;
        return units.size();
    };
    const bool trace = getenv("HX_TRACE") != nullptr;
    const auto t_entry = std::chrono::steady_clock::now();
    auto now_ms = [&]() { return std::chrono::duration<double, std::milli>(std::chrono::steady_clock::now() - t_entry).count(); };
    auto traced_upload = [&](size_t u) -> int {
        const double t0 = now_ms();
        const int rc = upload(u);
        if (trace) {
            const Sweep &w = sweeps[units[u].k];
            fprintf(stderr, "[hx] multi: sweep %zu (job %d, spin %d, %d comps) slab %d staged %.0f -> %.0f ms\n", units[u].k, w.job, spins[w.job], w.nb, units[u].slab, t0, now_ms());
        }
        return rc;
    };
    const size_t first_up = next_upload((size_t)-1);
    if (first_up < units.size()) HX_TRY(traced_upload(first_up));
    for (size_t u = 0; u < units.size(); ++u) {
        const size_t k = units[u].k;
        const Sweep &w = sweeps[k];
        const int slab = units[u].slab;
        if (uidx[u] >= 0) HX_HIP(hipStreamWaitEvent(rt().stream, unit_up[uidx[u] % NEV], 0));
        bool done = true;
        if (slab < 0) {
            const double *src = hidx[k] >= 0 ? pl->stage[hidx[k] % NST].as<double>() : maps[w.job] + (size_t)w.c0 * pl->npix;
            HX_TRY(analysis_batch(pl, spins[w.job], w.nb, src, valm[w.job].as<double2>() + (size_t)w.c0 * pl->nlm, vrw.as<double>(), vpw.as<double>(),
                                  vfl[w.job].as<double>(), 0));
        } else {
            if (slab == 0) HX_TRY(analysis_stream_start(ss[k]));
            HX_TRY(analysis_stream_slab(ss[k], slab));
            done = slab + 1 == ss[k].nslab;
            if (done) HX_TRY(analysis_stream_end(ss[k]));
        }
        if (done && hidx[k] >= 0) HX_HIP(hipEventRecord(pl->stage_done[hidx[k] % NST], rt().stream));
        if (trace) fprintf(stderr, "[hx] multi: sweep %zu slab %d queued at %.0f ms\n", k, slab, now_ms());
        if (uidx[u] >= 0) {
            const size_t q = next_upload(u);
            if (q < units.size()) HX_TRY(traced_upload(q));
        }
    }
    for (int j = 0; j < njobs; ++j) HX_TRY(valm[j].finish());
    if (trace) fprintf(stderr, "[hx] multi: everything queued at %.0f ms\n", now_ms());
    HX_HIP(hipStreamSynchronize(rt().stream));
    if (trace) fprintf(stderr, "[hx] multi: done at %.0f ms\n", now_ms());
    return HX_OK;
}

extern "C" int hx_map2alm(hx_plan *pl, int spin, int ncomp, const double *maps, double *alms,
                          const double *ring_weights, const double *pix_weights, const double *fl, int niter)
{
    HX_TRY(ensure_ready());
    HX_TRY(check_sht_args(pl, spin, ncomp, maps, alms, true));
    if (niter < 0) return fail(HX_ERR_ARG, "niter < 0");
    InView vmaps, vrw, vpw, vfl;
    OutView valms;
    if (niter == 0 && !is_device_ptr(maps) && copy_stream() != nullptr && !analysis_generic_spin(spin))
        return map2alm_multi_impl(pl, 1, &spin, &ncomp, &maps, nullptr, &alms, ring_weights, pix_weights, &fl);
    HX_TRY(vmaps.bind(maps, sizeof(double) * (size_t)ncomp * pl->npix));
    HX_TRY(vrw.bind(ring_weights, sizeof(double) * pl->nrp));
    HX_TRY(vpw.bind(pix_weights, sizeof(double) * (size_t)pl->npix));
    HX_TRY(classify_pixel_weights(pl, vpw.as<double>()));
    HX_TRY(vfl.bind(fl, sizeof(double) * (pl->lmax + 1)));
    HX_TRY(valms.bind(alms, sizeof(double2) * (size_t)ncomp * pl->nlm));
    DevBuf &resid = pl->resid_maps;
    if (niter > 0) HX_TRY(resid.alloc(sizeof(double) * (size_t)analysis_max_batch(spin, ncomp) * pl->npix));
    for (int c0 = 0, nb = 0; c0 < ncomp; c0 += nb) {
        nb = analysis_next_batch(spin, ncomp - c0);
        const double *dm = vmaps.as<double>() + (size_t)c0 * pl->npix;
        double2 *da = valms.as<double2>() + (size_t)c0 * pl->nlm;
        HX_TRY(analysis_batch(pl, spin, nb, dm, da, vrw.as<double>(), vpw.as<double>(), niter == 0 ? vfl.as<double>() : nullptr, 0));
        for (int it = 0; it < niter; ++it) {
            HX_TRY(synthesis_batch(pl, spin, nb, da, resid.as<double>(), dm));
            HX_TRY(analysis_batch(pl, spin, nb, resid.as<double>(), da, vrw.as<double>(), vpw.as<double>(), nullptr, 1));
        }
        if (niter > 0 && fl) HX_TRY(apply_fl(pl, nb, da, vfl.as<double>()));
    }
    HX_TRY(valms.finish());
    if (vmaps.tmp.p || vrw.tmp.p || vpw.tmp.p || vfl.tmp.p || valms.tmp.p) {
        HX_HIP(hipStreamSynchronize(rt().stream));
        return HX_OK;
    }
    return finish_call();
}

extern "C" int hx_map2alm_multi(hx_plan *pl, int njobs, const int *spins, const int *ncomps, const double *const *maps, double *const *alms,
                                const double *ring_weights, const double *pix_weights, const double *const *fls)
{
    return map2alm_multi_impl(pl, njobs, spins, ncomps, maps, nullptr, alms, ring_weights, pix_weights, fls);
}

extern "C" int hx_map2alm_list(hx_plan *pl, int nmaps, const int *spins, const double *const *maps, double *const *alms,
                               const double *ring_weights, const double *pix_weights, const double *fl0, const double *fl2, int niter)
{
    HX_TRY(ensure_ready());
    if (!pl || nmaps < 1 || !spins || !maps || !alms || niter < 0) return fail(HX_ERR_ARG, "hx_map2alm_list: bad arguments");
    std::vector<const double *> comps[2];
    std::vector<int> owner[2];
    for (int i = 0; i < nmaps; ++i) {
        if (spins[i] != 0 && spins[i] != 2) return fail(HX_ERR_UNSUPPORTED, "spin-%d maps not yet supported", spins[i]);
        if (!maps[i] || !alms[i]) return fail(HX_ERR_ARG, "hx_map2alm_list: null map or alm %d", i);
        const int g = spins[i] ? 0 : 1;
        comps[g].push_back(maps[i]);
        if (spins[i]) comps[g].push_back(maps[i] + pl->npix);
        owner[g].push_back(i);
    }
    int jspin[2], jn[2], nj = 0;
    const double *jmaps[2], *jfl[2];
    const double *const *jcomp[2];
    double *jalm[2];
    DevBuf out[2];
    for (int g = 0; g < 2; ++g) {
        if (comps[g].empty()) continue;
        HX_TRY(out[g].alloc(sizeof(double2) * comps[g].size() * (size_t)pl->nlm));
        jspin[nj] = g == 0 ? 2 : 0; jn[nj] = (int)comps[g].size(); jmaps[nj] = comps[g][0]; jcomp[nj] = comps[g].data();
        jalm[nj] = out[g].as<double>(); jfl[nj] = g == 0 ? fl2 : fl0;
        ++nj;
    }
    if (niter == 0) {
        HX_TRY(map2alm_multi_impl(pl, nj, jspin, jn, jmaps, jcomp, jalm, ring_weights, pix_weights, jfl));
    } else {
        InView vrw, vpw;
        HX_TRY(vrw.bind(ring_weights, sizeof(double) * pl->nrp));
        HX_TRY(vpw.bind(pix_weights, sizeof(double) * (size_t)pl->npix));
        for (int j = 0; j < nj; ++j) {
            DevBuf in;
            HX_TRY(in.alloc(sizeof(double) * (size_t)jn[j] * pl->npix));
            HX_TRY(gather_components(in.as<double>(), jn[j], pl->npix, [&](int c) { return jcomp[j][c]; }, nullptr));
            HX_TRY(hx_map2alm(pl, jspin[j], jn[j], in.as<double>(), jalm[j], vrw.as<double>(), vpw.as<double>(), jfl[j], niter));
            HX_HIP(hipStreamSynchronize(rt().stream));
        }
    }
    for (int g = 0; g < 2; ++g) {
        const int cpu = g == 0 ? 2 : 1;
        for (size_t u = 0; u < owner[g].size(); ++u) {
            const size_t bytes = sizeof(double2) * (size_t)cpu * pl->nlm;
            const char *src = (const char *)out[g].p + u * bytes;
            double *dst = alms[owner[g][u]];
            if (is_device_ptr(dst)) HX_HIP(hipMemcpyAsync(dst, src, bytes, hipMemcpyDeviceToDevice, rt().stream));
            else HX_TRY(copy_d2h(dst, src, bytes));
        }
    }
    HX_HIP(hipStreamSynchronize(rt().stream));
    return HX_OK;
}
```

heracles_amd/csrc/hx_plan.hip:

```cpp
#include <algorithm>
#include <cmath>

#include "hx_sht_common.h"

namespace hx {
__global__ void k_init_norm0(int lmax, double2 *__restrict__ coef, double *__restrict__ alpha)
{
    const int t = blockIdx.x * blockDim.x + threadIdx.x;
    const int m = t >> 1, par = t & 1;
    if (m > lmax) return;
    const double dm = m;
    auto a = [dm](double l) { return sqrt((4.0 * l * l - 1.0) / (l * l - dm * dm)); };
    double al = 1.0;
    for (int l = m + par; l <= lmax; l += 2) {
        const double dl = l;
        const double a1 = a(dl + 1.0), a2 = a(dl + 2.0);
        const double A = a1 * a2;
        double B = -a2 / a1;
        if (l > m) {
            const double a0 = a(dl);
            B -= a2 * a1 / (a0 * a0);
        }
        const double an = 0.25 * a2 * a1 / al;
        coef[almidx(lmax, l, m)] = make_double2(A * al / an, B * al / an);
        alpha[almidx(lmax, l, m)] = al;
        al = an;
    }
}

__global__ void k_init_norm2(int lmax, double2 *__restrict__ coef, double *__restrict__ alpha)
{
    const int m = blockIdx.x * blockDim.x + threadIdx.x;
    if (m > lmax) return;
    const int l0 = m > 2 ? m : 2;
    double am1 = 1.0, a0 = 1.0;
    for (int l = l0; l <= lmax; ++l) {
        alpha[almidx(lmax, l, m)] = a0;
        if (l == lmax) break;
        const double k = l, lp = l + 1.0, dm = m, dn = -2.0;
        const double den = k * sqrt((lp * lp - dm * dm) * (lp * lp - dn * dn));
        const double r1 = sqrt((2.0 * k + 3.0) / (2.0 * k + 1.0));
        const double p = r1 * (2.0 * k + 1.0) * k * lp / den;
        const double q = -r1 * (2.0 * k + 1.0) * dm * dn / den;
        double a1 = 1.0;
        if (l > l0) {
            const double r2 = sqrt((2.0 * k + 3.0) / (2.0 * k - 1.0));
            const double r = r2 * lp * sqrt((k * k - dm * dm) * (k * k - dn * dn)) / den;
            a1 = r * am1;
        }
        coef[almidx(lmax, l + 1, m)] = make_double2(p * a0 / a1, q * a0 / a1);
        am1 = a0;
        a0 = a1;
    }
}

__global__ void k_init_norm_s(int lmax, int s, double2 *__restrict__ coef, double *__restrict__ alpha)
{
    const int m = blockIdx.x * blockDim.x + threadIdx.x;
    if (m > lmax) return;
    const int l0 = m > s ? m : s;
    double am1 = 1.0, a0 = 1.0;
    for (int l = l0; l <= lmax; ++l) {
        alpha[almidx(lmax, l, m)] = a0;
        if (l == lmax) break;
        const double k = l, lp = l + 1.0, dm = m, dn = -(double)s;
        const double den = k * sqrt((lp * lp - dm * dm) * (lp * lp - dn * dn));
        const double r1 = sqrt((2.0 * k + 3.0) / (2.0 * k + 1.0));
        const double p = r1 * (2.0 * k + 1.0) * k * lp / den;
        const double q = -r1 * (2.0 * k + 1.0) * dm * dn / den;
        double a1 = 1.0;
        if (l > l0) {
            const double r2 = sqrt((2.0 * k + 3.0) / (2.0 * k - 1.0));
            const double r = r2 * lp * sqrt((k * k - dm * dm) * (k * k - dn * dn)) / den;
            a1 = r * am1;
        }
        coef[almidx(lmax, l + 1, m)] = make_double2(p * a0 / a1, q * a0 / a1);
        am1 = a0;
        a0 = a1;
    }
}
}

using namespace hx;

PlanDev hx_plan::dev() const
{
    PlanDev P;
    P.nside = nside; P.lmax = lmax; P.nrp = nrp; P.nrp_pad = nrp_pad; P.twN = twN;
    P.npix = npix; P.ny = ny;
    P.z = z.as<double>(); P.omz = omz.as<double>(); P.sth = sth.as<double>(); P.rwdef = rwdef.as<double>();
    P.nsub = nsub.as<int>(); P.shifted = shifted.as<int>();
    P.startN = startN.as<long long>(); P.startS = startS.as<long long>(); P.bhat_off = bhat_off.as<long long>();
    P.tw = tw.as<double2>(); P.bhat = bhat.as<double2>();
    P.mfac = mfac.as<double>(); P.kfac2 = kfac2.as<double>();
    P.rec0 = nullptr; P.rec2 = nullptr;
    P.wnorm = wnorm; P.hsrc = hsrc; P.hsrc_stride = hsrc_stride; P.hN = eqN;
    P.nssrc = nssrc; P.ns_m0 = ns_m0; P.ns_ms = m_step;
    return P;
}

static int plan_tables(hx_plan *pl)
{
    const int lmax = pl->lmax;
    std::vector<double2> tw(std::max(pl->twN / 2, 64));
    for (int k = 0; k < (int)tw.size(); ++k) {
        long double a = -2.0L * 3.141592653589793238462643383279502884L * k / pl->twN;
        tw[k].x = (double)cosl(a); tw[k].y = (double)sinl(a);
    }
    std::vector<double> mfac(lmax + 1), kfac2(lmax + 3, 0.0);
    {
        long double p = 1.0L;
        for (int m = 0; m <= lmax; ++m) {
            if (m > 0) p *= (2.0L * m - 1.0L) / (2.0L * m);
            long double v = sqrtl((2.0L * m + 1.0L) / (4.0L * 3.141592653589793238462643383279502884L) * p);
            mfac[m] = (double)((m & 1) ? -v : v);
        }
        long double k = 1.0L;
        for (int m = 2; m <= lmax + 2; ++m) {
            if (m > 2) k *= sqrtl((2.0L * m) * (2.0L * m - 1.0L) / ((m - 2.0L) * (m + 2.0L))) / 2.0L;
            kfac2[m] = (double)k;
        }
    }
    HX_TRY(upload(pl->tw, tw));
    HX_TRY(upload(pl->mfac, mfac));
    HX_TRY(upload(pl->kfac2, kfac2));
    hx_plan::SpinData *sd = nullptr;
    return spin_data(pl, 0, false, &sd);
}

extern "C" hx_plan *hx_plan_create(int nside, int lmax, int max_comp)
{
    if (ensure_ready() != HX_OK) return nullptr;
    if (nside < 1 || lmax < 0 || max_comp < 1) {
        set_error("hx_plan_create: bad argument");
        return nullptr;
    }
    hx_plan *pl = new hx_plan;
    pl->nside = nside; pl->lmax = lmax; pl->max_comp = max_comp;
    pl->npix = 12LL * nside * nside;
    pl->nrp = 2 * nside;
    pl->nrp_pad = (pl->nrp + 63) / 64 * 64;
    pl->nlm = (long long)(lmax + 1) * (lmax + 2) / 2;
    pl->wnorm = 4.0 * M_PI / (double)pl->npix;
    const long long ns = nside, ncap = 2 * ns * (ns - 1);
    std::vector<double> z(pl->nrp), omz(pl->nrp), sth(pl->nrp), rw(pl->nrp, 1.0);
    std::vector<int> nsub(pl->nrp), shifted(pl->nrp);
    std::vector<long long> sN(pl->nrp), sS(pl->nrp);
    const double fact2 = 4.0 / (double)pl->npix, fact1 = (double)(2 * ns) * fact2;
    int maxM = 1;
    for (int rp = 0; rp < pl->nrp; ++rp) {
        const int i = rp + 1;
        if (i < nside) {
            double tmp = (double)i * (double)i * fact2;
            z[rp] = 1.0 - tmp; omz[rp] = tmp; sth[rp] = sqrt(tmp * (2.0 - tmp));
            nsub[rp] = i; sN[rp] = 2LL * i * (i - 1); shifted[rp] = 1;
        } else {
            z[rp] = (double)(2 * nside - i) * fact1; omz[rp] = 1.0 - z[rp];
            sth[rp] = sqrt((1.0 - z[rp]) * (1.0 + z[rp]));
            nsub[rp] = nside; sN[rp] = ncap + (long long)(i - nside) * 4 * ns;
            shifted[rp] = ((i - nside) & 1) == 0;
        }
        sS[rp] = i == 2 * nside ? -1 : pl->npix - sN[rp] - 4LL * nsub[rp];
        maxM = std::max(maxM, fft_size_for(nsub[rp]));
    }
    pl->ny = sN[pl->nrp - 1] + 4LL * nsub[pl->nrp - 1];
    pl->twN = std::max(maxM, 2);
    pl->h_sth = sth; pl->h_z = z; pl->h_nsub = nsub; pl->h_startN = sN; pl->h_startS = sS;
    int rc = HX_OK;
    auto chk = [&](int r) { if (rc == HX_OK) rc = r; };
    chk(upload(pl->z, z)); chk(upload(pl->omz, omz)); chk(upload(pl->sth, sth)); chk(upload(pl->rwdef, rw));
    chk(upload(pl->nsub, nsub)); chk(upload(pl->shifted, shifted));
    chk(upload(pl->startN, sN)); chk(upload(pl->startS, sS));
    if (rc != HX_OK || plan_tables(pl) != HX_OK || ring_fft_plan_init(pl, nsub, sN, sS) != HX_OK) { delete pl; return nullptr; }
    if (hipStreamSynchronize(rt().stream) != hipSuccess || hipGetLastError() != hipSuccess) {
        set_error("hx_plan_create: table initialisation failed");
        delete pl;
        return nullptr;
    }
    return pl;
}

hx_plan *hx::plan_create_equiangular(int N, int lmax)
{
    if (N < 4 || (N & 3) || lmax < 0 || 2 * lmax + 1 >= N) {
        set_error("equiangular plan: N=%d lmax=%d", N, lmax);
        return nullptr;
    }
    hx_plan *pl = new hx_plan;
    pl->nside = 0; pl->lmax = lmax; pl->max_comp = 16;
    pl->npix = 0; pl->ny = 0;
    pl->eqN = N;
    pl->wnorm = 1.0 / N;
    pl->nrp = N / 4;
    pl->nrp_pad = (pl->nrp + 63) / 64 * 64;
    pl->nlm = (long long)(lmax + 1) * (lmax + 2) / 2;
    std::vector<double> z(pl->nrp), omz(pl->nrp), sth(pl->nrp), rw(pl->nrp, 1.0);
    for (int r = 0; r < pl->nrp; ++r) {
        const long double t = 2.0L * 3.141592653589793238462643383279502884L * (r + 0.5L) / N;
        const long double sh = sinl(0.5L * t);
        z[r] = (double)cosl(t); omz[r] = (double)(2.0L * sh * sh); sth[r] = (double)sinl(t);
    }
    pl->h_sth = sth; pl->h_z = z;
    pl->twN = 2;
    int rc = HX_OK;
    auto chk = [&](int r) { if (rc == HX_OK) rc = r; };
    chk(upload(pl->z, z)); chk(upload(pl->omz, omz)); chk(upload(pl->sth, sth)); chk(upload(pl->rwdef, rw));
    if (rc != HX_OK || plan_tables(pl) != HX_OK || hipStreamSynchronize(rt().stream) != hipSuccess) { delete pl; return nullptr; }
    return pl;
}

extern "C" void hx_plan_destroy(hx_plan *plan)
{
    if (!plan) return;
    if (rt().ready) (void)hipStreamSynchronize(rt().stream);
    for (int i = 0; i < hx_plan::NSTAGE; ++i) {
        if (plan->stage_done[i]) (void)hipEventDestroy(plan->stage_done[i]);
    }
    for (int i = 0; i < hx_plan::NUNIT_EV; ++i)
        if (plan->unit_up[i]) (void)hipEventDestroy(plan->unit_up[i]);
    delete plan;
}

extern "C" int hx_plan_release_scratch(hx_plan *pl)
{
    if (!pl) return fail(HX_ERR_ARG, "hx_plan_release_scratch: null plan");
    if (rt().ready) {
        HX_HIP(hipStreamSynchronize(rt().stream));
        if (rt().copy) HX_HIP(hipStreamSynchronize(rt().copy));
    }
    for (int i = 0; i < hx_plan::NSTAGE; ++i) pl->stage[i].release();
    pl->resid_maps.release();
    pl->Y.release();
    pl->F.release();
    pl->partial.release();
    pl->syn_tab.release();
    return HX_OK;
}

extern "C" int64_t hx_plan_scratch_bytes(const hx_plan *pl)
{
    if (!pl) return 0;
    size_t spin_tables = 0;
    for (const auto &kv : pl->spins) spin_tables += kv.second.cn.bytes + kv.second.al.bytes;
    return (int64_t)(pl->stage[0].bytes + pl->stage[1].bytes + pl->stage[2].bytes + pl->resid_maps.bytes + pl->Y.bytes + pl->F.bytes + pl->partial.bytes +
                     pl->bhat.bytes + pl->syn_tab.bytes + spin_tables);
}

extern "C" int hx_plan_last_chunks(const hx_plan *pl) { return pl ? pl->last_chunks : 0; }

namespace hx {
int spin_data(hx_plan *pl, int spin, bool generic, hx_plan::SpinData **out)
{
    const int lmax = pl->lmax, s = spin;
    if (generic ? (s < 1 || s > lmax) : (s != 0 && s != 2)) return fail(HX_ERR_ARG, "spin_data: spin %d at lmax %d", s, lmax);
    hx_plan::SpinData &sd = pl->spins[{s, generic}];
    *out = &sd;
    if (sd.cn.p && sd.al.p && (sd.kf.p || !generic)) return HX_OK;
    if (generic) {
        std::vector<double> kf(lmax + 1);
        const long double fourpi = 4.0L * 3.141592653589793238462643383279502884L;
        long double k = 1.0L;
        for (int m = s; m <= lmax; ++m) {
            if (m > s) k *= sqrtl((2.0L * m) * (2.0L * m - 1.0L) / ((long double)(m - s) * (m + s))) / 2.0L;
            const long double v = k * sqrtl((2.0L * m + 1.0L) / fourpi);
            kf[m] = (double)((m & 1) ? -v : v);
        }
        k = sqrtl((2.0L * s + 1.0L) / fourpi);
        for (int m = s - 1; m >= 0; --m) {
            k *= sqrtl((long double)(s + m + 1) / (s - m)) / 2.0L;
            kf[m] = (double)k;
        }
        for (double v : kf)
            if (!std::isfinite(v)) return fail(HX_ERR_UNSUPPORTED, "spin-%d values: the seeds of the recursion leave the range of a double", s);
        HX_TRY(upload(sd.kf, kf));
    }
    hipStream_t st = rt().stream;
    HX_TRY(sd.cn.alloc(sizeof(double2) * (pl->nlm + TABLE_PAD)));
    HX_TRY(sd.al.alloc(sizeof(double) * (pl->nlm + TABLE_PAD)));
    HX_HIP(hipMemsetAsync(sd.cn.p, 0, sizeof(double2) * (pl->nlm + TABLE_PAD), st));
    HX_HIP(hipMemsetAsync(sd.al.p, 0, sizeof(double) * (pl->nlm + TABLE_PAD), st));
    double2 *cn = sd.cn.as<double2>();
    double *al = sd.al.as<double>();
    if (generic) hipLaunchKernelGGL(k_init_norm_s, dim3((lmax + 64) / 64), dim3(64), 0, st, lmax, s, cn, al);
    else if (s == 2) hipLaunchKernelGGL(k_init_norm2, dim3((lmax + 64) / 64), dim3(64), 0, st, lmax, cn, al);
    else hipLaunchKernelGGL(k_init_norm0, dim3((2 * (lmax + 1) + 63) / 64), dim3(64), 0, st, lmax, cn, al);
    HX_HIP(hipGetLastError());
    return HX_OK;
}

static int ring_mlim(int lmax, int spin, double sth, double cth)
{
    double ofs = lmax * 0.01;
    if (ofs < 100.) ofs = 100.;
    double b = -2 * spin * fabs(cth);
    double t1 = lmax * sth + ofs;
    double c = (double)spin * spin - t1 * t1;
    double discr = b * b - 4 * c;
    if (discr <= 0) return lmax;
    double res = (-b + sqrt(discr)) / 2.;
    if (res > lmax) res = lmax;
    return (int)(res + 0.5);
}

int task_set(hx_plan *pl, int spin, bool generic, int blocks, hx_plan::TaskSet **out)
{
    if (spin < 0 || blocks < 1) return fail(HX_ERR_ARG, "task_set: %d ring blocks per task of spin %d", blocks, spin);
    std::map<int, hx_plan::TaskSet> &store = pl->spins[{spin, generic}].tasks;
    const auto it = store.find(blocks);
    if (it != store.end()) {
        *out = &it->second;
        return HX_OK;
    }
    hx_plan::TaskSet &ts = store[blocks];
    const int lmax = pl->lmax;
    const int nrb = (pl->nrp + RBLK - 1) / RBLK;
    ts.of_m.assign(lmax + 1, MTasks{0, 0});
    ts.rows_before_m.assign(lmax + 2, 0);
    ts.arow.assign(lmax + 2, 0);
    long long rows = 0, arows = 0;
    std::vector<int> mlim(pl->nrp);
    for (int rp = 0; rp < pl->nrp; ++rp) mlim[rp] = ring_mlim(lmax, spin, pl->h_sth[rp], pl->h_z[rp]);
    for (int m = 0; m <= lmax; ++m) {
        ts.rows_before_m[m] = rows;
        ts.arow[m] = arows;
        const int l0 = std::max(m, spin);
        if (l0 <= lmax) arows += (long long)LBLK * ((lmax - l0) / LBLK + 1);
        ts.of_m[m].first = (int)ts.tasks.size();
        if (l0 <= lmax) {
            int first = (int)(std::lower_bound(mlim.begin(), mlim.end(), m) - mlim.begin());
            if (first >= pl->nrp) first = pl->nrp - 1;
            for (int rb = first / RBLK; rb < nrb; rb += blocks) {
                LegTask t;
                t.m = m; t.rb0 = rb; t.nrb = std::min(blocks, nrb - rb); t.pad = 0; t.pout = rows;
                rows += (long long)LBLK * ((lmax - l0) / LBLK + 1);
                ts.tasks.push_back(t);
            }
        }
        ts.of_m[m].count = (int)ts.tasks.size() - ts.of_m[m].first;
    }
    ts.rows_before_m[lmax + 1] = rows;
    ts.arow[lmax + 1] = arows;
    int rc = upload(ts.d_tasks, ts.tasks);
    if (rc == HX_OK) rc = upload(ts.d_of_m, ts.of_m);
    if (rc == HX_OK) rc = upload(ts.d_arow, ts.arow);
    if (rc != HX_OK) store.erase(blocks);
    *out = rc == HX_OK ? &ts : nullptr;
    return rc;
}

int synth_mlim(hx_plan *pl, int spin, const int **mlim)
{
    hx_plan::SpinData *sd = nullptr;
    HX_TRY(spin_data(pl, spin, false, &sd));
    if (!sd->syn_mlim.p) {
        std::vector<int> h(pl->nrp_pad, -1);
        for (int rp = 0; rp < pl->nrp; ++rp) {
            const int last = std::min(rp / RBLK * RBLK + RBLK - 1, pl->nrp - 1);
            h[rp] = std::min(pl->lmax, ring_mlim(pl->lmax, spin, pl->h_sth[last], pl->h_z[last]));
        }
        HX_TRY(upload(sd->syn_mlim, h));
    }
    *mlim = sd->syn_mlim.as<int>();
    return HX_OK;
}
}
```

heracles_amd/csrc/hx_sht_common.h:

```cpp
#pragma once
#include <map>
#include <vector>

#include "hx_common.h"
#include "hx_fft_core.h"

namespace hx {

typedef double double4_t __attribute__((ext_vector_type(4)));

constexpr int LBLK = 32;
constexpr int NCOL = 16;
constexpr int TABLE_PAD = 512;
constexpr int NGMAX = 2;
constexpr int RBLK = 32;
constexpr double SC_BIG = 0x1p+300, SC_SMALL = 0x1p-300;
constexpr int SPIN_ANY = -1;

struct LegTask {
    int m;
    int rb0;
    int nrb;
    int pad;
    long long pout;
};

struct MTasks {
    int first, count;
};

struct alignas(16) RingDesc {
    long long sN, sS, bhat_off;
    int n, rp;
};
struct PlanDev {
    int nside, lmax, nrp, nrp_pad, twN;
    long long npix, ny;
    const double *z, *omz, *sth, *rwdef;
    const int *nsub, *shifted;
    const long long *startN, *startS, *bhat_off;
    const double2 *tw, *bhat;
    const double *mfac, *kfac2;
    const double2 *rec0;
    const double4 *rec2;
    double wnorm;
    const double2 *hsrc;
    long long hsrc_stride;
    int hN;
    const double4 *const *nssrc;
    int ns_m0, ns_ms;
};

__host__ __device__ inline long long almidx(int lmax, int l, int m)
{
    return (long long)m * (2 * lmax + 1 - m) / 2 + l;
}

__device__ inline double2 expipi(double x)
{
    double s, c;
    sincospi(x, &s, &c);
    return make_double2(c, s);
}

struct SVal {
    double v;
    int e;
};

__device__ inline void snorm_small(SVal &s)
{
    if (s.v != 0.0)
        while (fabs(s.v) < SC_SMALL) {
            s.v *= SC_BIG;
            s.e -= 1;
        }
}

template <int SB>
__device__ inline void sval_rebase(double &v, int &e)
{
    static_assert(300 % SB == 0, "the step must divide 300");
    if (SB != 300) {
        constexpr double big = SB == 100 ? 0x1p+100 : SB == 150 ? 0x1p+150 : SB == 75 ? 0x1p+75 : SB == 60 ? 0x1p+60 : 0x1p+50;
        static_assert(SB == 300 || SB == 100 || SB == 150 || SB == 75 || SB == 60 || SB == 50, "unsupported step");
        e *= 300 / SB;
        if (v != 0.0)
            while (fabs(v) < 1.0 / big) {
                v *= big;
                e -= 1;
            }
    }
}

__device__ inline SVal spow(double x, int n)
{
    SVal r = {1.0, 0}, b = {x, 0};
    while (n) {
        if (n & 1) {
            r.v *= b.v;
            r.e += b.e;
            snorm_small(r);
        }
        n >>= 1;
        if (n) {
            b.v *= b.v;
            b.e *= 2;
            snorm_small(b);
        }
    }
    return r;
}

__device__ inline double sval_true(double v, int e)
{
    return e == 0 ? v : (e == -1 ? v * SC_SMALL : 0.0);
}

__device__ inline void spin2_seeds(int m, double sth, double omx, double kfac2m, SVal &sp, SVal &sm)
{
    const int l0 = m > 2 ? m : 2;
    const double opx = 2.0 - omx;
    const double nrm = sqrt((2.0 * l0 + 1.0) / (4.0 * M_PI));
    if (m == 0) {
        const double d = 0.61237243569579452455 * sth * sth;
        sp.v = sm.v = nrm * d; sp.e = sm.e = 0;
    } else if (m == 1) {
        sp.v = nrm * (-0.5 * omx * sth); sp.e = 0;
        sm.v = nrm * (0.5 * opx * sth);  sm.e = 0;
    } else {
        SVal b = spow(sth, m - 2);
        b.v *= kfac2m * nrm * ((m & 1) ? -1.0 : 1.0);
        sp.v = b.v * (0.25 * omx * omx); sp.e = b.e;
        sm.v = b.v * (0.25 * opx * opx); sm.e = b.e;
    }
    snorm_small(sp);
    snorm_small(sm);
}

__device__ inline void spin_seeds(int s, int m, double sth, double omx, double kfsm, SVal &sp, SVal &sm)
{
    const double opx = 2.0 - omx;
    SVal b = spow(sth, m >= s ? m - s : s - m);
    b.v *= kfsm;
    const int n = m >= s ? s : m;
    const SVal ps = spow(0.5 * omx, n), pc = spow(0.5 * opx, n);
    sp.v = b.v * ps.v; sp.e = b.e + ps.e;
    sm.v = b.v * pc.v; sm.e = b.e + pc.e;
    if (m < s) {
        if (m & 1) sp.v = -sp.v;
        if (s & 1) sm.v = -sm.v;
    }
    snorm_small(sp);
    snorm_small(sm);
}

#ifdef __HIPCC__
using namespace hxfft;
struct RingAtM {
    double2 ph;
    long long i0, i1;
    int hasS;
};

__device__ inline void ring_modes_ns(const PlanDev &P, const double2 *__restrict__ Y, int c, int rp, int m,
                                     const RingAtM &r, double2 &FN, double2 &FS, int s = 0)
{
    if (P.nssrc) {
        const double4 v = P.nssrc[c][(long long)((m - P.ns_m0) / P.ns_ms) * P.nrp_pad + rp];
        FN = make_double2(v.x, v.y);
        FS = make_double2(v.z, v.w);
        return;
    }
    if (P.hsrc) {
        const double w = r.ph.x;
        const double2 *h = P.hsrc + (long long)c * P.hsrc_stride + (long long)m * P.hN;
        const double sg = ((m + s) & 1) ? -w : w;
        const double2 a = h[rp], b = h[P.hN - 1 - rp], cN = h[P.hN / 2 - 1 - rp], d = h[P.hN / 2 + rp];
        FN = make_double2(w * a.x + sg * b.x, w * a.y + sg * b.y);
        FS = make_double2(w * cN.x + sg * d.x, w * cN.y + sg * d.y);
        return;
    }
    const double2 *Yc = Y + (long long)c * P.ny;
    const double2 a = Yc[r.i0], b = cconj(Yc[r.i1]);
    const double2 xn = cscale(cadd(a, b), 0.5);
    const double2 xs = mul_mi(cscale(csub(a, b), 0.5));
    FN = cmul(xn, r.ph);
    FS = r.hasS ? cmul(xs, r.ph) : make_double2(0.0, 0.0);
}

__device__ inline RingAtM ring_at_m_of(const PlanDev &P, int r, int m, const double *__restrict__ rw)
{
    RingAtM q;
    const bool live = r < P.nrp;
    const double w = live ? (rw ? rw[r] : 1.0) * P.wnorm : 0.0;
    q.ph = make_double2(w, 0.0);
    q.i0 = q.i1 = 0;
    q.hasS = 0;
    if (live && !P.hsrc) {
        const int n = P.nsub[r], nphi = 4 * n;
        const int mm = m % nphi, mc = (nphi - mm) % nphi;
        q.i0 = P.startN[r] + (long long)(mm & 3) * n + (mm >> 2);
        q.i1 = P.startN[r] + (long long)(mc & 3) * n + (mc >> 2);
        if (P.shifted[r]) q.ph = cscale(expipi(-(double)(m % (2 * nphi)) / (double)nphi), w);
        q.hasS = P.startS[r] >= 0;
    }
    return q;
}

template <class TW>
__device__ __forceinline__ void lds_fft_pass_dif(double2 *buf, int M, int K, int h, int gt, int gn, TW tw, int twN)
{
    switch (K) {
    case 4:
_Pragma("unroll 1")
        for (int i = gt; i < (M >> 4); i += gn) dif_pass_butterfly<4>(buf, i, h, tw, twN); break;
    case 3:
_Pragma("unroll 1")
        for (int i = gt; i < (M >> 3); i += gn) dif_pass_butterfly<3>(buf, i, h, tw, twN); break;
    case 2:
_Pragma("unroll 1")
        for (int i = gt; i < (M >> 2); i += gn) dif_pass_butterfly<2>(buf, i, h, tw, twN); break;
    default: for (int i = gt; i < (M >> 1); i += gn) dif_pass_butterfly<1>(buf, i, h, tw, twN); break;
    }
}
template <class TW>
__device__ __forceinline__ void lds_fft_pass_dit_inv(double2 *buf, int M, int K, int h, int gt, int gn, TW tw, int twN)
{
    switch (K) {
    case 4:
_Pragma("unroll 1")
        for (int i = gt; i < (M >> 4); i += gn) dit_inv_pass_butterfly<4>(buf, i, h, tw, twN); break;
    case 3:
_Pragma("unroll 1")
        for (int i = gt; i < (M >> 3); i += gn) dit_inv_pass_butterfly<3>(buf, i, h, tw, twN); break;
    case 2:
_Pragma("unroll 1")
        for (int i = gt; i < (M >> 2); i += gn) dit_inv_pass_butterfly<2>(buf, i, h, tw, twN); break;
    default: for (int i = gt; i < (M >> 1); i += gn) dit_inv_pass_butterfly<1>(buf, i, h, tw, twN); break;
    }
}
template <class TW>
__device__ __forceinline__ void lds_fft_dif(double2 *buf, int M, TW tw, int twN, int gt, int gn, bool skip_last = false)
{
    const int p = ilog2(M), np = fft_sched_np(p);
    int h = M;
    for (int a = 0; a < np - (skip_last ? 1 : 0); ++a) {
        const int K = fft_sched_k(p, a);
        h >>= K;
        lds_fft_pass_dif(buf, M, K, h, gt, gn, tw, twN);
        __syncthreads();
    }
}
template <class TW>
__device__ __forceinline__ void lds_fft_dit_inv(double2 *buf, int M, TW tw, int twN, int gt, int gn, bool skip_first = false)
{
    const int p = ilog2(M), np = fft_sched_np(p);
    int h = 1;
    for (int a = np - 1; a >= 0; --a) {
        const int K = fft_sched_k(p, a);
        if (!(skip_first && a == np - 1)) {
            lds_fft_pass_dit_inv(buf, M, K, h, gt, gn, tw, twN);
            __syncthreads();
        }
        h <<= K;
    }
}
template <class TW>
__device__ __forceinline__ void lds_fft_dif(double2 *buf, int M, TW tw, int twN) { lds_fft_dif(buf, M, tw, twN, (int)threadIdx.x, (int)blockDim.x); }
template <class TW>
__device__ __forceinline__ void lds_fft_dit_inv(double2 *buf, int M, TW tw, int twN) { lds_fft_dit_inv(buf, M, tw, twN, (int)threadIdx.x, (int)blockDim.x); }

constexpr int TW_HI_MAX = 128;
__device__ inline TwFactored load_tw_factored(double2 *hi, double2 *lo, const double2 *__restrict__ tw, int twN)
{
    for (int i = threadIdx.x; i < (twN >= 128 ? twN / 128 : 1); i += blockDim.x) hi[i] = tw[i * 64];
    for (int i = threadIdx.x; i < 64; i += blockDim.x) lo[i] = tw[i];
    TwFactored f;
    f.hi = hi;
    f.lo = lo;
    return f;
}

#endif

template <class T>
inline int upload(DevBuf &b, const std::vector<T> &v)
{
    HX_TRY(b.alloc(sizeof(T) * (v.size() > 0 ? v.size() : 1)));
    if (!v.empty()) HX_HIP(hipMemcpy(b.p, v.data(), sizeof(T) * v.size(), hipMemcpyHostToDevice));
    return HX_OK;
}

}

struct hx_plan {
    int nside = 0, lmax = 0, max_comp = 0;
    int nrp = 0, nrp_pad = 0, twN = 1;
    int fft_cap = 8192;
    int last_chunks = 0;
    int eqN = 0;
    double wnorm = 0.0;
    const double2 *hsrc = nullptr;
    long long hsrc_stride = 0;
    const double4 *const *nssrc = nullptr;
    int ns_m0 = 0;
    int m_lo = 0, m_hi = -1, m_step = 1;
    long long npix = 0, ny = 0, nlm = 0;
    size_t lds_fft = 0;
    hx::DevBuf z, omz, sth, rwdef, nsub, shifted, startN, startS, bhat_off, tw, bhat, mfac, kfac2;
    std::vector<double> h_sth, h_z;
    std::vector<int> h_nsub;
    std::vector<long long> h_startN, h_startS;
    struct TaskSet {
        std::vector<hx::LegTask> tasks;
        std::vector<hx::MTasks> of_m;
        std::vector<long long> rows_before_m;
        std::vector<long long> arow;
        hx::DevBuf d_tasks, d_of_m, d_arow;
    };
    struct SpinData {
        hx::DevBuf cn, al, kf;
        hx::DevBuf syn_mlim;
        hx::DevBuf syn_boff;
        std::map<int, TaskSet> tasks;
    };
    std::map<std::pair<int, bool>, SpinData> spins;
    struct FftClass { int M, first, count, big; };
    std::vector<FftClass> fft_classes;
    hx::DevBuf fft_rp_list;
    hx::DevBuf fft_desc;
    std::vector<int> h_fft_rp_list;
    hx::DevBuf Y, F, partial, d_dbg, resid_maps, pw_sym;
    hx::DevBuf syn_tab;
    const double *pw_checked = nullptr;
    int pw_mode = 0;
    static constexpr int NSTAGE = 3;
    hx::DevBuf stage[NSTAGE];
    hipEvent_t stage_done[NSTAGE] = {nullptr, nullptr, nullptr};
    static constexpr int NUNIT_EV = 4;
    hipEvent_t unit_up[NUNIT_EV] = {nullptr, nullptr, nullptr, nullptr};
    hx::PlanDev dev() const;
};

namespace hx {
hx_plan *plan_create_equiangular(int N, int lmax);
int spin_data(hx_plan *pl, int spin, bool generic, hx_plan::SpinData **out);
int task_set(hx_plan *pl, int spin, bool generic, int blocks, hx_plan::TaskSet **out);
int synth_mlim(hx_plan *pl, int spin, const int **mlim);
int ring_fft_plan_init(hx_plan *pl, const std::vector<int> &nsub, const std::vector<long long> &sN, const std::vector<long long> &sS);
int launch_ring_subdft_maps(hx_plan *pl, int nb, const double *d_maps, const double *d_pw, double2 *Y, int rp_lo = 0, int rp_hi = 0x7fffffff);
int launch_ring_subdft_spectra(hx_plan *pl, int nc, const double2 *zin, double *pixout, const double *ref);
int classify_pixel_weights(hx_plan *pl, const double *d_pw);
int synthesis_batch(hx_plan *pl, int spin, int nb, const double2 *d_alms, double *d_maps, const double *d_ref);
int check_sht_args(hx_plan *pl, int spin, int ncomp, const void *a, const void *b, bool any_spin = false);
int one_set_task_blocks(int spin);
int flop_task_blocks(int spin);
int analysis_batch(hx_plan *pl, int spin, int nb, const double *d_maps, double2 *d_alms, const double *d_rw,
                   const double *d_pw, const double *d_fl, int add);
bool analysis_generic_spin(int spin);
inline bool plan_generic_spin(const hx_plan *pl, int spin) { return (pl->hsrc || (pl->nside >= 1 && !pl->nssrc)) && analysis_generic_spin(spin); }
int analysis_max_comp(int spin);
int analysis_next_batch(int spin, int remaining);
int analysis_max_batch(int spin, int ncomp);
struct StreamSweep {
    hx_plan *pl = nullptr;
    int spin = 0, nb = 0, nslab = 0;
    const double *d_maps = nullptr, *d_rw = nullptr, *d_pw = nullptr, *d_fl = nullptr;
    double2 *d_alms = nullptr;
    std::vector<int> rp_edge;
    DevBuf d_of_m;
    hx_plan::SpinData *sd = nullptr;
    hx_plan::TaskSet *ts = nullptr;
};
bool analysis_can_stream(hx_plan *pl, int spin, int nb);
int analysis_stream_plan(hx_plan *pl, int spin, int nb, int nslab, StreamSweep &s);
int analysis_stream_start(StreamSweep &s);
int analysis_stream_slab(StreamSweep &s, int k);
int analysis_stream_end(StreamSweep &s);
int launch_valu_chunk(hx_plan *pl, int spin, const hx_plan::SpinData &sd, hx_plan::TaskSet &ts, int m0, int m1, int c0, const double *d_rw, bool generic = false);
int valu_task_blocks(int spin);
int valu_partial_cols(int spin);
int valu_operand_doubles(int spin);
int valu_exec_flops(unsigned long long *v, bool reset);
int synth_valu_max_units(int spin);
int synth_valu_task_blocks(int spin, int units);
int launch_synth_valu(hx_plan *pl, int spin, int units, const hx_plan::SpinData &sd, hx_plan::TaskSet &ts, const double2 *d_alm, double *d_Fv, bool generic = false);
int synth_duo_max_units(int spin);
int synth_duo_rowlen(int spin, int units);
size_t synth_duo_table_bytes(hx_plan *pl, int spin, int units);
int synth_duo_min_units(int spin);
int launch_synth_duo(hx_plan *pl, int spin, int units, hx_plan::SpinData &sd, hx_plan::TaskSet &ts, const double2 *d_alm, double *d_tab, double *d_Fv);
}
```

heracles_amd/sht.py:

```python

from __future__ import annotations

import numpy as np

from . import _lib


def nlm(lmax: int) -> int:
    return (lmax + 1) * (lmax + 2) // 2


def _is_tensor(a) -> bool:
    return hasattr(a, "data_ptr") and not isinstance(a, np.ndarray)


class Plan:

    def __init__(self, nside: int, lmax: int, max_comp: int = 8):
        L = _lib.load()
        _lib.ensure_init()
        self.nside, self.lmax = int(nside), int(lmax)
        self.npix = 12 * self.nside**2
        self.nlm = nlm(self.lmax)
        self._h = L.hx_plan_create(self.nside, self.lmax, int(max_comp))
        if not self._h:
            raise _lib.HxError(-1, L.hx_last_error().decode(errors="replace"))

    def close(self):
        if getattr(self, "_h", None):
            _lib.load().hx_plan_destroy(self._h)
            self._h = None

    def release_scratch(self):
        _lib.check(_lib.load().hx_plan_release_scratch(self._h))

    def __del__(self):
        try:
            self.close()
        except Exception:
            pass

    @property
    def scratch_bytes(self) -> int:
        return int(_lib.load().hx_plan_scratch_bytes(self._h))

    @property
    def last_chunks(self) -> int:
        return int(_lib.load().hx_plan_last_chunks(self._h))

    def mfma_flops(self, spin, ncomp):
        import ctypes

        out = ctypes.c_double(0.0)
        _lib.check(_lib.load().hx_plan_mfma_flops(self._h, int(spin), int(ncomp), ctypes.byref(out)))
        return out.value

    def executed_flops(self, spin, ncomp):
        import ctypes

        out = (ctypes.c_double * 2)()
        _lib.check(_lib.load().hx_plan_executed_flops(self._h, int(spin), int(ncomp), out))
        return out[0], out[1]

    def _out_like(self, ref, shape, complex_):
        if _is_tensor(ref):
            import torch

            return torch.empty(shape, dtype=torch.complex128 if complex_ else torch.float64,
                               device=ref.device)
        return np.empty(shape, dtype=np.complex128 if complex_ else np.float64)

    @staticmethod
    def _prep(a, dtype):
        if a is None:
            return None
        if _is_tensor(a):
            return a.contiguous()
        return np.ascontiguousarray(a, dtype=dtype)

    def map2alm(self, maps, spin=0, *, ring_weights=None, pix_weights=None, fl=None,
                niter=0, out=None):
        maps = self._prep(maps, np.float64)
        lead = tuple(maps.shape[:-1])
        if maps.shape[-1] != self.npix:
            raise ValueError(f"map has {maps.shape[-1]} pixels, plan expects {self.npix}")
        ncomp = int(np.prod(lead)) if lead else 1
        if out is None:
            out = self._out_like(maps, lead + (self.nlm,), True)
        rw = self._prep(ring_weights, np.float64)
        pw = self._prep(pix_weights, np.float64)
        flv = self._prep(fl, np.float64)
        if flv is not None and flv.shape[-1] != self.lmax + 1:
            raise ValueError("fl must have lmax+1 entries")
        _lib.check(_lib.load().hx_map2alm(self._h, int(spin), ncomp, _lib.ptr(maps), _lib.ptr(out),
                                          _lib.ptr(rw), _lib.ptr(pw), _lib.ptr(flv), int(niter)))
        return out

    def map2alm_multi(self, jobs, *, ring_weights=None, pix_weights=None):
        import ctypes as C

        n = len(jobs)
        keep, outs = [], []
        spins, ncomps = (C.c_int * n)(), (C.c_int * n)()
        pm, pa, pf = (C.c_void_p * n)(), (C.c_void_p * n)(), (C.c_void_p * n)()
        for j, job in enumerate(jobs):
            maps, spin, out = job[0], job[1], job[2]
            fl = job[3] if len(job) > 3 else None
            maps = self._prep(maps, np.float64)
            if maps.shape[-1] != self.npix:
                raise ValueError(f"map has {maps.shape[-1]} pixels, plan expects {self.npix}")
            lead = tuple(maps.shape[:-1])
            nc = int(np.prod(lead)) if lead else 1
            if out is None:
                out = self._out_like(maps, lead + (self.nlm,), True)
            flv = self._prep(fl, np.float64)
            if flv is not None and flv.shape[-1] != self.lmax + 1:
                raise ValueError("fl must have lmax+1 entries")
            keep += [maps, flv]
            outs.append(out)
            spins[j], ncomps[j] = int(spin), nc
            pm[j], pa[j], pf[j] = _lib.ptr(maps), _lib.ptr(out), _lib.ptr(flv)
        rw = self._prep(ring_weights, np.float64)
        pw = self._prep(pix_weights, np.float64)
        _lib.check(_lib.load().hx_map2alm_multi(self._h, n, spins, ncomps, pm, pa, _lib.ptr(rw), _lib.ptr(pw), pf))
        return outs

    def map2alm_list(self, maps, spins, *, outs=None, ring_weights=None, pix_weights=None, fl0=None, fl2=None, niter=0, fls=None):
        spins = [int(s) for s in spins]
        if any(s < 0 for s in spins):
            raise NotImplementedError(f"spin-{min(spins)} maps not yet supported")
        listed = [i for i, s in enumerate(spins) if s in (0, 2)]
        res = [None] * len(spins)
        if listed:
            got = self._map2alm_list([maps[i] for i in listed], [spins[i] for i in listed],
                                     outs=None if outs is None else [outs[i] for i in listed], ring_weights=ring_weights,
                                     pix_weights=pix_weights, fl0=fl0, fl2=fl2, niter=niter)
            for i, a in zip(listed, got):
                res[i] = a
        for i, s in enumerate(spins):
            if s not in (0, 2):
                res[i] = self.map2alm(maps[i], s, ring_weights=ring_weights, pix_weights=pix_weights, fl=(fls or {}).get(s),
                                      niter=niter, out=None if outs is None else outs[i])
        return res

    def _map2alm_list(self, maps, spins, *, outs=None, ring_weights=None, pix_weights=None, fl0=None, fl2=None, niter=0):
        import ctypes as C

        n = len(maps)
        keep, res = [], []
        sp = (C.c_int * n)()
        pm, pa = (C.c_void_p * n)(), (C.c_void_p * n)()
        for i, (m, s) in enumerate(zip(maps, spins)):
            m = self._prep(m, np.float64)
            want = (self.npix,) if int(s) == 0 else (2, self.npix)
            if int(s) not in (0, 2):
                raise NotImplementedError(f"spin-{s} maps not yet supported")
            if tuple(m.shape) != want:
                raise ValueError(f"map {i} of spin {s} has shape {tuple(m.shape)}, expected {want}")
            out = outs[i] if outs is not None else self._out_like(m, want[:-1] + (self.nlm,), True)
            keep.append(m)
            res.append(out)
            sp[i] = int(s)
            pm[i], pa[i] = _lib.ptr(m), _lib.ptr(out)
        rw = self._prep(ring_weights, np.float64)
        pw = self._prep(pix_weights, np.float64)
        f0, f2 = self._prep(fl0, np.float64), self._prep(fl2, np.float64)
        for f in (f0, f2):
            if f is not None and f.shape[-1] != self.lmax + 1:
                raise ValueError("fl must have lmax+1 entries")
        _lib.check(_lib.load().hx_map2alm_list(self._h, n, sp, pm, pa, _lib.ptr(rw), _lib.ptr(pw), _lib.ptr(f0), _lib.ptr(f2), int(niter)))
        return res

    def alm2map(self, alms, spin=0, *, out=None):
        alms = self._prep(alms, np.complex128)
        lead = tuple(alms.shape[:-1])
        if alms.shape[-1] != self.nlm:
            raise ValueError(f"alm has {alms.shape[-1]} coefficients, plan expects {self.nlm}")
        ncomp = int(np.prod(lead)) if lead else 1
        if out is None:
            out = self._out_like(alms, lead + (self.npix,), False)
        _lib.check(_lib.load().hx_alm2map(self._h, int(spin), ncomp, _lib.ptr(alms), _lib.ptr(out)))
        return out


_plans: dict = {}


def get_plan(nside: int, lmax: int) -> Plan:
    key = (int(nside), int(lmax))
    if key not in _plans:
        _plans[key] = Plan(nside, lmax)
    return _plans[key]


def clear_plans():
    for p in _plans.values():
        p.close()
    _plans.clear()
```

include/hxsht.h:

```cpp
#ifndef HXSHT_H
#define HXSHT_H
#include <stdint.h>
#ifdef __cplusplus
extern "C" {
#endif

#define HX_OK 0
#define HX_ERR_ARG (-1)
#define HX_ERR_NO_DEVICE (-2)
#define HX_ERR_HIP (-3)
#define HX_ERR_MEM (-4)
#define HX_ERR_UNSUPPORTED (-5)

typedef struct hx_plan hx_plan;

const char *hx_version(void);
const char *hx_last_error(void);
int hx_device_count(void);
int hx_init(int device);
int hx_set_stream(void *stream);
void *hx_get_stream(void);
int hx_set_async(int on);
int hx_synchronize(void);
int hx_copy(void *dst, const void *src, int64_t bytes);
int hx_host_alloc(int64_t bytes, void **out);
int hx_host_free(void *p);

int hx_timer_start(void);
int hx_timer_stop(float *ms);
int hx_profile_enable(int on);
int hx_profile_reset(void);
int hx_profile_get(const char *name, int *launches, double *total_ms);

hx_plan *hx_plan_create(int nside, int lmax, int max_comp);
int hx_set_max_lds_fft(int points);
void hx_plan_destroy(hx_plan *plan);
int64_t hx_plan_scratch_bytes(const hx_plan *plan);
int hx_plan_release_scratch(hx_plan *plan);
int hx_set_scratch_budget(double bytes);
int hx_plan_last_chunks(const hx_plan *plan);
int hx_measure_peaks(double *out4);
double hx_measured_mfma_clock(void);
double hx_mixmat_gemm_clock(void);
int hx_plan_mfma_flops(hx_plan *plan, int spin, int ncomp, double *flops);
int hx_plan_executed_flops(hx_plan *plan, int spin, int ncomp, double *out2);
int hx_executed_flops(double *out2, int reset);

int hx_map2alm(hx_plan *plan, int spin, int ncomp, const double *maps, double *alms,
               const double *ring_weights, const double *pix_weights, const double *fl,
               int niter);
int hx_alm2map(hx_plan *plan, int spin, int ncomp, const double *alms, double *maps);
int hx_map2alm_multi(hx_plan *plan, int njobs, const int *spins, const int *ncomps, const double *const *maps, double *const *alms,
                     const double *ring_weights, const double *pix_weights, const double *const *fls);
int hx_map2alm_list(hx_plan *plan, int nmaps, const int *spins, const double *const *maps, double *const *alms,
                    const double *ring_weights, const double *pix_weights, const double *fl0, const double *fl2, int niter);

int64_t hx_ring_modes_size(const hx_plan *plan, int count);
int hx_ring_modes(hx_plan *plan, int ncomp, const double *maps, const double *pix_weights, const double *ring_weights, int nsets,
                  const int *m_first, const int *m_count, int m_step, double *const *outs);
int hx_legendre_from_modes(hx_plan *plan, int spin, int ncomp, const double *const *comp_modes, int m_first, int m_count, int m_step,
                           double *alms, const double *fl);

int hx_allgather_alms(void *comm, int nranks, const int64_t *counts, double *buf);

int hx_alm2cl_pairs(int ncomp, const int *lmax_i, const double *const *alms, int lmax_out,
                    int npairs, const int *pair_i, const int *pair_j, double *cls);
int hx_alm2cl_pairs_range(int ncomp, const int *lmax_i, const double *const *alms, int lmax_out, int npairs, const int *pair_i,
                          const int *pair_j, int m0, int m1, int mstep, double *cls);

int hx_gauss_legendre(int n, double *x, double *w);
int hx_gauss_legendre_dd(int n, double *x, double *w, double *xlo);

#define HX_MAX_MIX_SPIN 32
int hx_wigner_d_table(int lmax, int a, int b, int n, const double *x, double *out);

int hx_mixmat(const double *cl, int ncl, int l1max, int l2max, int l3max, int s1, int s2,
              double *out);
int hx_mixmat_eb(const double *cl, int ncl, int l1max, int l2max, int l3max, double *out);
int hx_mixmat_eb_spin(const double *cl, int ncl, int l1max, int l2max, int l3max, int s1, int s2, double *out);
int hx_mixmat_release(void);
int hx_release_caches(void);
int hx_fits_unpack_f64(int64_t nrows, int nc1, int nc2, int64_t s1, int64_t s2, int64_t srow, const void *table, double *array);
int hx_fits_pack_f64(int64_t nrows, int nc1, int nc2, int64_t s1, int64_t s2, int64_t srow, const double *array, void *table);

#define HX_FITS_MAX_COLUMNS 64
#define HX_FITS_DIRECT 1
int hx_fits_unpack_columns(int64_t nrows, int64_t width, int ncols, const int64_t *offsets, const char *types, const double *tscal,
                           const double *tzero, const void *table, double *const *columns, int flags);

int hx_region_maps(int64_t npix, int ncomp, const double *maps, const double *region, double k, double *out);
int hx_alm_subtract(int64_t n, const double *full, int nsub, const double *const *subs, double *out);

int hx_matvec(int n, int m, const double *M, int nvec, const double *x, double *y);

int hx_pinv(int n, int m, const double *M, double rcond, double *out, double *info);

typedef struct hx_mixctx hx_mixctx;
hx_mixctx *hx_mixctx_create(int l1max, int l2max, int l3max);
int hx_mixctx_apply(hx_mixctx *ctx, const double *cl, int ncl, int kind, double *out);
int hx_mixctx_apply_spin(hx_mixctx *ctx, const double *cl, int ncl, int s1, int s2, double *out);
void hx_mixctx_destroy(hx_mixctx *ctx);
int hx_mixctx_set_bins(hx_mixctx *ctx, int nbins, const int *which, const double *w, const double *norm);
int hx_mixctx_apply_binned(hx_mixctx *ctx, const double *cl, int ncl, int kind, double *out);
int hx_mixctx_apply_binned_spin(hx_mixctx *ctx, const double *cl, int ncl, int s1, int s2, double *out);
int hx_mixmat_batch(int nmask, const double *cls, int ncl, int l1max, int l2max, int l3max, const int *kinds,
                    double *const *out00, double *const *out02, double *const *outeb);

int hx_cl2corr(int lmax, int nspec, const double *cls, double *corrs);
int hx_corr2cl(int lmax, int nspec, const double *corrs, double *cls);

int hx_cl2corr_cols(int lmax, int nl, int ncol, const int *family, const double *a, double *xi);
int hx_corr2cl_cols(int lmax, int nl, int ncol, const int *family, const double *xi, double *b);
int hx_cl2corr_cols_spin(int lmax, int nl, int ncol, const int *pairs, const double *a, double *xi);
int hx_corr2cl_cols_spin(int lmax, int nl, int ncol, const int *pairs, const double *xi, double *b);
int hx_xi_ratio(int n, int ncol, const double *xi_d, const double *xi_num, const int *num_col, const double *xi_den, const int *den_col,
                const int *ndamp, double x0, double k, double *out);

int hx_alm_resample(int lmax_in, int lmax_out, int ncomp, const double *alm_in, double *alm_out);

typedef struct hx_pointsht hx_pointsht;
hx_pointsht *hx_pointsht_create(int lmax, double epsilon);
void hx_pointsht_destroy(hx_pointsht *ps);
int hx_pointsht_info(const hx_pointsht *ps, int *info4);
int hx_pointsht_adjoint(hx_pointsht *ps, int spin, int ncomp, int64_t npoints, const double *loc, const double *map, double *alm);
int hx_pointsht_synthesis(hx_pointsht *ps, int spin, int ncomp, int64_t npoints, const double *loc, const double *alm, double *map);
typedef struct hx_pointgrid hx_pointgrid;
hx_pointgrid *hx_pointsht_grids(hx_pointsht *ps, int spin, int ncomp, const double *alm);
int hx_pointgrid_gather(hx_pointgrid *g, int64_t npoints, const double *loc, double *map);
void hx_pointgrid_destroy(hx_pointgrid *g);

#define HX_MAP_ATOMIC 1
int hx_ang2pix_ring(int nside, int64_t n, const double *lon, const double *lat, int64_t *ipix);
int hx_map_values(int nside, int64_t n, const double *lon, const double *lat, int nval,
                  const double *values, double *maps, int flags);

int hx_ud_grade(int nside_in, int nside_out, int nmaps, const double *in, double *out);

int hx_reorder(int nside, int to_ring, int nmaps, const double *in, double *out);

typedef struct hx_catmap hx_catmap;
#define HX_CAT_POSITIONS 0
#define HX_CAT_SCALAR 1
#define HX_CAT_COMPLEX 2
#define HX_CAT_WEIGHTS 3
#define HX_CAT_MAX_FIELDS 8
#define HX_CAT_MAX_GROUPS 4
#define HX_CAT_MAX_COLUMNS 16
hx_catmap *hx_catmap_create(int64_t page_size, int ncols, int nfields, const int *desc, double *const *maps);
int hx_catmap_page(hx_catmap *ctx, int64_t n, const double *const *cols);
int hx_catmap_moments(hx_catmap *ctx, double *out, int64_t *bad);
int hx_catmap_finish(hx_catmap *ctx, int field, double norm, const double *vis);
void hx_catmap_destroy(hx_catmap *ctx);

typedef struct hx_catalm hx_catalm;
hx_catalm *hx_catalm_create(int64_t page_size, int ncols, int nfields, const int *desc, hx_pointsht *const *ps);
int hx_catalm_page(hx_catalm *ctx, int64_t n, const double *const *cols);
int hx_catalm_moments(hx_catalm *ctx, double *out, int64_t *bad);
int hx_catalm_finish(hx_catalm *ctx, int field, int spin, double norm, const double *vis_alm, double *alm);
void hx_catalm_destroy(hx_catalm *ctx);

typedef struct hx_catmap_sel hx_catmap_sel;
#define HX_CAT_MAX_SELECTIONS 32
#define HX_CAT_MAX_PREDICATES 64
#define HX_CAT_MAX_FILTERS 4
#define HX_CAT_EQ 0
#define HX_CAT_NE 1
#define HX_CAT_LT 2
#define HX_CAT_LE 3
#define HX_CAT_GT 4
#define HX_CAT_GE 5
#define HX_CAT_FILTER_INVALID 0
#define HX_CAT_FILTER_FOOTPRINT 1
hx_catmap_sel *hx_catmap_create_sel(int64_t page_size, int ncols, int nfields, const int *desc, int nsel, int npred, const int *preds,
                                    const double *pval, int nfilt, const int *filters, const double *const *footprints, double *const *maps);
int hx_catmap_page_sel(hx_catmap_sel *ctx, int64_t n, const double *const *cols, const uint32_t *mask);
int hx_catmap_moments_sel(hx_catmap_sel *ctx, double *out, int64_t *bad, int64_t *fcount);
int hx_catmap_finish_sel(hx_catmap_sel *ctx, int sel, int field, double norm, const double *vis);
void hx_catmap_destroy_sel(hx_catmap_sel *ctx);

int64_t hx_pixel_weights_size(int nside);
int hx_pixel_weights_expand(int nside, int64_t ncompressed, const double *compressed, double *weights);
int hx_pixel_weights_solve(hx_plan *plan, int lmax, double epsilon, int itmax, double *compressed_out, int *iterations,
                           double *rel_gradient, double *max_residual);

int hx_cov_gram(int n, int n1, int n2, const double *x, const double *y, double alpha, double *out);
int hx_cov_delete2(int njk, int m, int N, const double *c0, const double *c1, const double *c2, const int *pairs, const int *perm,
                   int nb, const int *bstart, double alpha, double *out);
int hx_cov_shrink_sums(int n, int N, const double *x, const double *target, int64_t ldt, double *out);

#ifdef __cplusplus
}
#endif
#endif
```

Before: 428.0.

## Cache Legendre recurrence lead-in state via scout kernel and resume analysis

Adds a one-time scout pass of the Legendre analysis kernel that runs the recurrence without MFMA work, finds the first block where each task's values become significant, and stores the recurrence state there together with that block index. Later analysis launches zero the skipped partial rows and resume the recurrence from the stored state, so the lead-in recurrence steps are not recomputed on every transform. This is on by default for spin 2, and spin 0 is opt-in. The cost is a device table of up to 8 GiB (limited to a tenth of free memory), an extra scout launch the first time, and extra branching in the kernel.

```diff
diff --git a/heracles_amd/_lib.py b/heracles_amd/_lib.py
--- a/heracles_amd/_lib.py
+++ b/heracles_amd/_lib.py
@@ -19,7 +19,7 @@
     "hx_version", "hx_last_error", "hx_device_count", "hx_init", "hx_set_stream",
     "hx_get_stream", "hx_set_async", "hx_synchronize", "hx_timer_start", "hx_timer_stop",
     "hx_profile_enable", "hx_profile_reset", "hx_profile_get", "hx_plan_create", "hx_set_max_lds_fft",
-    "hx_plan_destroy", "hx_plan_scratch_bytes", "hx_plan_release_scratch", "hx_set_scratch_budget", "hx_plan_last_chunks", "hx_plan_mfma_flops", "hx_plan_executed_flops", "hx_executed_flops", "hx_measure_peaks", "hx_measured_mfma_clock", "hx_map2alm", "hx_map2alm_multi", "hx_map2alm_list", "hx_alm2map", "hx_copy",
+    "hx_plan_destroy", "hx_plan_scratch_bytes", "hx_plan_release_scratch", "hx_plan_set_leadin_resume", "hx_plan_set_leadin_cap", "hx_set_scratch_budget", "hx_plan_last_chunks", "hx_plan_mfma_flops", "hx_plan_executed_flops", "hx_executed_flops", "hx_measure_peaks", "hx_measured_mfma_clock", "hx_map2alm", "hx_map2alm_multi", "hx_map2alm_list", "hx_alm2map", "hx_copy",
     "hx_alm2cl_pairs", "hx_alm2cl_pairs_range", "hx_gauss_legendre", "hx_gauss_legendre_dd", "hx_wigner_d_table", "hx_mixmat",
     "hx_mixmat_eb", "hx_mixmat_eb_spin", "hx_mixmat_batch", "hx_mixctx_create", "hx_mixctx_apply", "hx_mixctx_apply_spin", "hx_mixctx_destroy", "hx_mixctx_set_bins", "hx_mixctx_apply_binned", "hx_mixctx_apply_binned_spin", "hx_cl2corr", "hx_corr2cl", "hx_cl2corr_cols", "hx_corr2cl_cols", "hx_cl2corr_cols_spin", "hx_corr2cl_cols_spin", "hx_xi_ratio", "hx_ang2pix_ring", "hx_map_values", "hx_ud_grade", "hx_reorder", "hx_matvec", "hx_pinv", "hx_alm_resample", "hx_region_maps", "hx_alm_subtract", "hx_fits_unpack_f64", "hx_fits_pack_f64", "hx_fits_unpack_columns",
     "hx_pointsht_create", "hx_pointsht_destroy", "hx_pointsht_info", "hx_pointsht_adjoint",
@@ -72,6 +72,8 @@
         L.hx_plan_scratch_bytes.argtypes = [vp]
         L.hx_plan_scratch_bytes.restype = C.c_int64
         L.hx_plan_release_scratch.argtypes = [vp]
+        L.hx_plan_set_leadin_resume.argtypes = [vp, i]
+        L.hx_plan_set_leadin_cap.argtypes = [vp, C.c_int64]
         L.hx_set_scratch_budget.argtypes = [C.c_double]
         L.hx_plan_last_chunks.argtypes = [vp]
         L.hx_plan_mfma_flops.argtypes = [vp, i, i, C.POINTER(C.c_double)]
diff --git a/heracles_amd/csrc/hx_analysis.hip b/heracles_amd/csrc/hx_analysis.hip
--- a/heracles_amd/csrc/hx_analysis.hip
+++ b/heracles_amd/csrc/hx_analysis.hip
@@ -32,6 +32,9 @@
     const long long *__restrict__ arow;
     long long arow0;
     int add_all;
+    const double *__restrict__ leadin;
+    LegTask *tasks_out;
+    double *leadin_out;
 };
 
 constexpr int COMB_NXCD = 8, COMB_XG = 4;
@@ -253,7 +256,7 @@
     }
 }
 
-template <int SPIN, int NG, int NBX, int NSUB = 1>
+template <int SPIN, int NG, int NBX, int NSUB = 1, bool SCOUT = false, bool RESUME = SPIN == 2>
 __global__ __launch_bounds__(256, 2) void k_legendre_duo(LegParams A, const double2 *__restrict__ coefn)
 {
     using C = PipeCfg<SPIN>;
@@ -268,7 +271,7 @@
     constexpr int TW = NSUB * DSZ > 2048 ? NSUB * DSZ : 2048;
     static_assert(NG >= 1 && NG <= 2 && TW * NW * 8 <= 81920, "two work-groups per CU");
     static_assert(SPIN == 0 || HALF_F, "spin 2: the lambda- chain carries (-1)^(l + m) lambda- (one operand row, wave-uniform coefficients)");
-    __shared__ double tile[NW][TW];
+    __shared__ double tile[NW][SCOUT ? 2 : TW];
     __shared__ int lead_in[2][NW];
     const PlanDev &P = A.P;
     const int m = A.m0 + blockIdx.x * A.ms, lmax = P.lmax;
@@ -289,14 +292,25 @@
     };
     int n_mf = 0, n_rec = 0;
     if (DUO_PRIO) __builtin_amdgcn_s_setprio(3);
-    for (int ti = 0; ti < mt.count; ++ti) {
-        const LegTask task = A.tasks[mt.first + ti];
+    const int ti0 = SCOUT ? (int)blockIdx.y : 0, tis = SCOUT ? (int)gridDim.y : 1;
+    for (int ti = ti0; ti < mt.count; ti += tis) {
+        const LegTask task = SCOUT ? A.tasks_out[mt.first + ti] : A.tasks[mt.first + ti];
         first_group = ti == 0 && !A.add_all;
+        const int bres = (RESUME && !SCOUT && A.leadin) ? task.pad : 0;
         int tid = threadIdx.x;
         asm volatile("; ring group" : "+v"(tid));
         const int w = tid >> 6, lane = tid & 63;
         const int ai = lane & 15, ak = lane >> 4;
-        if (ti) __syncthreads();
+        if (ti != ti0) __syncthreads();
+        if (!SCOUT && bres > 0) {
+            if (first_group) {
+                double2 *z = reinterpret_cast<double2 *>(A.partial + orow * A.pcol);
+                const long long nz = (long long)bres * LBLK * A.pcol / 2;
+                for (long long i = tid; i < nz; i += 256) z[i] = make_double2(0.0, 0.0);
+                asm volatile("s_waitcnt vmcnt(0)" ::: "memory");
+            }
+            if (bres >= nblk) continue;
+        }
 
         const int rbi = SPIN == 0 ? 2 * w + (lane >> 5) : w;
         const int rpl = (task.rb0 + rbi) * RBLK + (lane & 31);
@@ -309,7 +323,7 @@
         for (int sp = 0; sp < NPAIR; ++sp) {
             const int op = SPIN == 0 ? 0 : sp & 1, q = SPIN == 0 ? sp : sp >> 1;
             const int rbq = SPIN == 0 ? 2 * w + (q >> 3) : w;
-            const bool on = rbq < task.nrb;
+            const bool on = !SCOUT && rbq < task.nrb;
             const long long row = (long long)blockIdx.x * P.nrp_pad + (task.rb0 + rbq) * RBLK + pipe_rho(q & 7, ak);
             if (HALFB) {
                 const double *f = A.F + (row * NOP + op) * A.ncol;
@@ -333,7 +347,15 @@
         int sc[NCH];
 #pragma unroll
         for (int c = 0; c < NCH; ++c) { vc[c] = 0.0; vp[c] = 0.0; sc[c] = -100; }
-        if (valid) {
+        if (bres > 0) {
+            const double *st = A.leadin + (long long)(mt.first + ti) * (NCH * 640) + tid;
+#pragma unroll
+            for (int c = 0; c < NCH; ++c) {
+                vc[c] = st[c * 640];
+                vp[c] = st[c * 640 + 256];
+                sc[c] = reinterpret_cast<const int *>(st + c * 640 + 512 - tid)[tid];
+            }
+        } else if (valid) {
             if (SPIN == 0) {
                 SVal a = spow(P.sth[rpl], m);
                 a.v *= P.mfac[m];
@@ -390,7 +412,7 @@
                     }
                     cur[k] = rec_step(RMM, SPIN == 0 ? ((kk & 1) ? NCH - 1 : 0) : 0, SPIN == 0 ? kk >> 1 : kk, tq);
                 }
-                if (RM >= 2) {
+                if (RM >= 2 && !SCOUT) {
 #pragma unroll
                     for (int j = 0; j < HB / 2; ++j)
                         *reinterpret_cast<double2 *>(tw + pipe_tile_idx(lane, h * (HB / 2) + j)) = make_double2(cur[2 * j], cur[2 * j + 1]);
@@ -419,15 +441,22 @@
         const int fcol = tid & 15, fch = (tid >> 4) & 7, fpos = (tid >> 7) & 1;
         const int frow = (fch >> 1) + 8 * (fch & 1);
         const int qrow = tid / (4 * NXA), qcol = tid % (4 * NXA);
-        double *pgrp = A.partial + (orow + 2 * frow + fpos) * A.pcol + fcol;
-        double *pquad = A.partial + (orow + 2 * qrow) * A.pcol + NG * NCOL + qcol;
-        double2 cnext[2] = {cfm[0], cfm[16]};
+        double *pgrp = A.partial + (orow + (long long)bres * LBLK + 2 * frow + fpos) * A.pcol + fcol;
+        double *pquad = A.partial + (orow + (long long)bres * LBLK + 2 * qrow) * A.pcol + NG * NCOL + qcol;
+        double2 cnext[2] = {cfm[bres * LBLK], cfm[bres * LBLK + 16]};
         bool started = first_group;
         int nflush = 0;
-        for (int b0 = 0; b0 < nblk; b0 += NSUB) {
+        int woke = nblk;
+        double svc[NCH], svp[NCH];
+        int ssc[NCH];
+        for (int b0 = bres; b0 < nblk; b0 += NSUB) {
             double4_t acc[NSUB][NG][2];
             double accx[NSUB][NXA][2];
             bool mine = false;
+            if (SCOUT) {
+#pragma unroll
+                for (int c = 0; c < NCH; ++c) { svc[c] = vc[c]; svp[c] = vp[c]; ssc[c] = sc[c]; }
+            }
 #pragma unroll
             for (int sub = 0; sub < NSUB; ++sub) {
                 const int b = b0 + sub;
@@ -451,7 +480,7 @@
                 cnext[1] = cfm[(b + 1) * LBLK + 16];
                 n_rec = __builtin_amdgcn_readfirstlane(n_rec + 1);
                 mine = mine || rm >= 2;
-                if (rm >= 2) {
+                if (!SCOUT && rm >= 2) {
                     n_mf = __builtin_amdgcn_readfirstlane(n_mf + 1);
                     if (DUO_PRIO) __builtin_amdgcn_s_setprio(0);
                     constexpr int PF = 3;
@@ -515,6 +544,17 @@
                 }
             }
             const bool two = NSUB > 1 && b0 + 1 < nblk;
+            if (SCOUT) {
+                if (lane == 0) lead_in[nflush & 1][w] = mine ? 1 : 0;
+                lds_barrier();
+                const int4 fl = *reinterpret_cast<const int4 *>(&lead_in[nflush & 1][0]);
+                ++nflush;
+                if (__builtin_amdgcn_readfirstlane(fl.x | fl.y | fl.z | fl.w) != 0) {
+                    woke = b0;
+                    break;
+                }
+                continue;
+            }
             if (!started) {
                 if (lane == 0) lead_in[nflush & 1][w] = mine ? 1 : 0;
                 lds_barrier();
@@ -567,8 +607,20 @@
             pquad += (long long)NSUB * LBLK * A.pcol;
             lds_barrier();
         }
-    }
-    if ((threadIdx.x & 63) == 0) {
+        if (SCOUT) {
+            if (woke > 0 && woke < nblk) {
+                double *st = A.leadin_out + (long long)(mt.first + ti) * (NCH * 640) + tid;
+#pragma unroll
+                for (int c = 0; c < NCH; ++c) {
+                    st[c * 640] = svc[c];
+                    st[c * 640 + 256] = svp[c];
+                    reinterpret_cast<int *>(st + c * 640 + 512 - tid)[tid] = ssc[c];
+                }
+            }
+            if (tid == 0) A.tasks_out[mt.first + ti].pad = woke;
+        }
+    }
+    if (!SCOUT && (threadIdx.x & 63) == 0) {
         atomicAdd(&g_exec_flops[0], (unsigned long long)n_mf * (32ull * (NG * 2048ull + NBX * 512ull)));
         atomicAdd(&g_exec_flops[1], (unsigned long long)n_rec * (64ull * LBLK * 4ull));
     }
@@ -703,6 +755,13 @@
 {
     const dim3 db(256);
     const int key = sh.ng * 10 + sh.nbx;
+    if (SPIN == 0 && A.leadin) {
+        if (key == 10) hipLaunchKernelGGL((k_legendre_duo<0, 1, 0, 2, false, true>), pgrid, db, 0, st, A, cn);
+        else if (key == 11) hipLaunchKernelGGL((k_legendre_duo<0, 1, 1, 2, false, true>), pgrid, db, 0, st, A, cn);
+        else if (key == 20) hipLaunchKernelGGL((k_legendre_duo<0, 2, 0, 1, false, true>), pgrid, db, 0, st, A, cn);
+        else return fail(HX_ERR_ARG, "legendre analysis: no two-group kernel for %d groups + %d blocks", sh.ng, sh.nbx);
+        return HX_OK;
+    }
     if (key == 10) hipLaunchKernelGGL((k_legendre_duo<SPIN, 1, 0, 2>), pgrid, db, 0, st, A, cn);
     else if (key == 11) hipLaunchKernelGGL((k_legendre_duo<SPIN, 1, 1, 2>), pgrid, db, 0, st, A, cn);
     else if (key == 20 && SPIN == 2) hipLaunchKernelGGL((k_legendre_duo<2, 2, 0, 2>), pgrid, db, 0, st, A, cn);
@@ -714,6 +773,45 @@
     return HX_OK;
 }
 
+constexpr long long LEADIN_CAP_BYTES = 8LL << 30;
+static int leadin_table(hx_plan *pl, int spin, hx_plan::SpinData &sd, hx_plan::TaskSet &ts, const double **tab)
+{
+    *tab = nullptr;
+    if (pl->leadin_resume < (spin == 0 ? 2 : 1) || ts.tasks.empty() || ts.leadin_skip) return HX_OK;
+    if (ts.d_leadin.p) {
+        *tab = ts.d_leadin.as<double>();
+        return HX_OK;
+    }
+    const size_t per_task = (size_t)(spin == 0 ? PipeCfg<0>::NCH : PipeCfg<2>::NCH) * 640 * sizeof(double);
+    const size_t bytes = ts.tasks.size() * per_task;
+    size_t cap = (size_t)(pl->leadin_cap > 0 ? pl->leadin_cap : LEADIN_CAP_BYTES), fr = 0, tot = 0;
+    if (hipMemGetInfo(&fr, &tot) == hipSuccess) cap = std::min(cap, fr / 10);
+    else (void)hipGetLastError();
+    if (bytes > cap) {
+        ts.leadin_skip = true;
+        return HX_OK;
+    }
+    if (ts.d_leadin.alloc(bytes) != HX_OK) {
+        (void)hipGetLastError();
+        ts.leadin_skip = true;
+        return HX_OK;
+    }
+    LegParams A;
+    A.P = pl->dev(); A.tasks = nullptr; A.F = nullptr; A.partial = nullptr;
+    A.m0 = 0; A.ms = 1; A.row0 = 0; A.ng = 1; A.ncol = NCOL; A.pcol = NCOL;
+    A.of_m = ts.d_of_m.as<MTasks>(); A.arow = ts.d_arow.as<long long>(); A.arow0 = 0; A.add_all = 1;
+    A.leadin = nullptr; A.tasks_out = ts.d_tasks.as<LegTask>(); A.leadin_out = ts.d_leadin.as<double>();
+    const dim3 grid((unsigned)(pl->lmax + 1), 8), db(256);
+    if (spin == 0) hipLaunchKernelGGL((k_legendre_duo<0, 1, 0, 2, true>), grid, db, 0, rt().stream, A, sd.cn.as<double2>());
+    else hipLaunchKernelGGL((k_legendre_duo<2, 1, 0, 2, true>), grid, db, 0, rt().stream, A, sd.cn.as<double2>());
+    if (hipGetLastError() != hipSuccess) {
+        ts.d_leadin.release();
+        return fail(HX_ERR_HIP, "leadin_table: the scout launch failed");
+    }
+    *tab = ts.d_leadin.as<double>();
+    return HX_OK;
+}
+
 static void launch_alm_reduce(hx_plan *pl, int spin, hx_plan::TaskSet &ts, long long row0, int m0, int ms, int nm, int nb, int ng, int pcol,
                               const double *d_fl, int add, double2 *d_alms, const double *al)
 {
@@ -729,7 +827,7 @@
 
 template <int SPIN>
 static int launch_chunk(hx_plan *pl, hx_plan::SpinData &sd, hx_plan::TaskSet &ts, int m0, int m1, int nb, const SweepShape &sh, const double *d_rw,
-                        const double *d_fl, int add, double2 *d_alms)
+                        const double *d_fl, int add, double2 *d_alms, const double *leadin)
 {
     const int ng = sh.ng + (sh.nbx > 0 ? 1 : 0), ncol = sh.ncol;
     const int pcol = sweep_pcol(sh);
@@ -751,6 +849,7 @@
         A.m0 = m0; A.ms = ms; A.row0 = ts.rows_before_m[m0]; A.ng = ng; A.ncol = ncol; A.pcol = pcol;
         A.of_m = ts.d_of_m.as<MTasks>(); A.arow = ts.d_arow.as<long long>(); A.arow0 = ts.arow[m0]; A.add_all = 0;
         A.tasks = ts.d_tasks.as<LegTask>();
+        A.leadin = leadin; A.tasks_out = nullptr; A.leadin_out = nullptr;
         HX_TRY(launch_duo<SPIN>(sh, dim3((unsigned)nm), st, A, sd.cn.as<double2>()));
     }
     {
@@ -851,11 +950,13 @@
     }
     std::vector<std::pair<int, int>> chunks;
     HX_TRY(plan_m_chunks(pl, (double)pl->nrp_pad * analysis_f_rows(spin) * sh.ncol * sizeof(double), ts->arow, sweep_pcol(sh) * sizeof(double), chunks));
+    const double *leadin = nullptr;
+    HX_TRY(leadin_table(pl, spin, *sd, *ts, &leadin));
     for (auto &ch : chunks) {
         if (spin == 0)
-            HX_TRY(launch_chunk<0>(pl, *sd, *ts, ch.first, ch.second, nb, sh, d_rw, d_fl, add, d_alms));
+            HX_TRY(launch_chunk<0>(pl, *sd, *ts, ch.first, ch.second, nb, sh, d_rw, d_fl, add, d_alms, leadin));
         else
-            HX_TRY(launch_chunk<2>(pl, *sd, *ts, ch.first, ch.second, nb, sh, d_rw, d_fl, add, d_alms));
+            HX_TRY(launch_chunk<2>(pl, *sd, *ts, ch.first, ch.second, nb, sh, d_rw, d_fl, add, d_alms, leadin));
     }
     return HX_OK;
 }
@@ -889,6 +990,7 @@
     HX_TRY(task_set(pl, spin, false, one_set_task_blocks(spin), &s.ts));
     hx_plan::TaskSet &ts = *s.ts;
     const SweepShape sh = sweep_shape(spin, nb);
+    s.leadin = nullptr;
     s.pl = pl; s.spin = spin; s.nb = nb;
     const int nrb = (pl->nrp + RBLK - 1) / RBLK;
     std::vector<double> cum(nrb + 1, 0.0);
@@ -926,6 +1028,8 @@
     return HX_OK;
 }
 
+int analysis_stream_leadin(StreamSweep &s) { return leadin_table(s.pl, s.spin, *s.sd, *s.ts, &s.leadin); }
+
 int analysis_stream_start(StreamSweep &s)
 {
     hx_plan *pl = s.pl;
@@ -959,6 +1063,7 @@
         A.P = P; A.tasks = ts.d_tasks.as<LegTask>(); A.F = pl->F.as<double>(); A.partial = pl->partial.as<double>();
         A.m0 = 0; A.ms = 1; A.row0 = 0; A.ng = ng; A.ncol = sh.ncol; A.pcol = sweep_pcol(sh);
         A.of_m = s.d_of_m.as<MTasks>() + (size_t)k * (lmax + 1); A.arow = ts.d_arow.as<long long>(); A.arow0 = 0; A.add_all = 1;
+        A.leadin = s.leadin; A.tasks_out = nullptr; A.leadin_out = nullptr;
         HX_TRY(launch_duo<SPIN>(sh, dim3((unsigned)nm), st, A, s.sd->cn.as<double2>()));
     }
     HX_HIP(hipGetLastError());
diff --git a/heracles_amd/csrc/hx_map2alm.hip b/heracles_amd/csrc/hx_map2alm.hip
--- a/heracles_amd/csrc/hx_map2alm.hip
+++ b/heracles_amd/csrc/hx_map2alm.hip
@@ -107,6 +107,8 @@
         ss[k].d_alms = valm[w.job].as<double2>() + (size_t)w.c0 * pl->nlm;
         ss[k].d_rw = vrw.as<double>(); ss[k].d_pw = vpw.as<double>(); ss[k].d_fl = vfl[w.job].as<double>();
     }
+    for (size_t k = 0; k < sweeps.size(); ++k)
+        if (sweeps[k].stream) HX_TRY(analysis_stream_leadin(ss[k]));
     struct Unit { size_t k; int slab; };
     std::vector<Unit> units;
     for (size_t k = 0; k < sweeps.size(); ++k) {
diff --git a/heracles_amd/csrc/hx_plan.hip b/heracles_amd/csrc/hx_plan.hip
--- a/heracles_amd/csrc/hx_plan.hip
+++ b/heracles_amd/csrc/hx_plan.hip
@@ -234,6 +234,27 @@
     pl->F.release();
     pl->partial.release();
     pl->syn_tab.release();
+    for (auto &sp : pl->spins)
+        for (auto &kv : sp.second.tasks) {
+            kv.second.d_leadin.release();
+            kv.second.leadin_skip = false;
+        }
+    return HX_OK;
+}
+
+extern "C" int hx_plan_set_leadin_resume(hx_plan *pl, int on)
+{
+    if (!pl) return fail(HX_ERR_ARG, "hx_plan_set_leadin_resume: null plan");
+    pl->leadin_resume = on < 0 ? 0 : (on > 2 ? 2 : on);
+    return HX_OK;
+}
+
+extern "C" int hx_plan_set_leadin_cap(hx_plan *pl, int64_t bytes)
+{
+    if (!pl || bytes < 0) return fail(HX_ERR_ARG, "hx_plan_set_leadin_cap: null plan or negative cap");
+    pl->leadin_cap = bytes;
+    for (auto &sp : pl->spins)
+        for (auto &kv : sp.second.tasks) kv.second.leadin_skip = false;
     return HX_OK;
 }
 
@@ -241,7 +262,10 @@
 {
     if (!pl) return 0;
     size_t spin_tables = 0;
-    for (const auto &kv : pl->spins) spin_tables += kv.second.cn.bytes + kv.second.al.bytes;
+    for (const auto &kv : pl->spins) {
+        spin_tables += kv.second.cn.bytes + kv.second.al.bytes;
+        for (const auto &ts : kv.second.tasks) spin_tables += ts.second.d_leadin.bytes;
+    }
     return (int64_t)(pl->stage[0].bytes + pl->stage[1].bytes + pl->stage[2].bytes + pl->resid_maps.bytes + pl->Y.bytes + pl->F.bytes + pl->partial.bytes +
                      pl->bhat.bytes + pl->syn_tab.bytes + spin_tables);
 }
diff --git a/heracles_amd/csrc/hx_sht_common.h b/heracles_amd/csrc/hx_sht_common.h
--- a/heracles_amd/csrc/hx_sht_common.h
+++ b/heracles_amd/csrc/hx_sht_common.h
@@ -306,6 +306,8 @@
     const double4 *const *nssrc = nullptr;
     int ns_m0 = 0;
     int m_lo = 0, m_hi = -1, m_step = 1;
+    int leadin_resume = 1;
+    long long leadin_cap = 0;
     long long npix = 0, ny = 0, nlm = 0;
     size_t lds_fft = 0;
     hx::DevBuf z, omz, sth, rwdef, nsub, shifted, startN, startS, bhat_off, tw, bhat, mfac, kfac2;
@@ -318,6 +320,8 @@
         std::vector<long long> rows_before_m;
         std::vector<long long> arow;
         hx::DevBuf d_tasks, d_of_m, d_arow;
+        hx::DevBuf d_leadin;
+        bool leadin_skip = false;
     };
     struct SpinData {
         hx::DevBuf cn, al, kf;
@@ -372,8 +376,10 @@
     DevBuf d_of_m;
     hx_plan::SpinData *sd = nullptr;
     hx_plan::TaskSet *ts = nullptr;
+    const double *leadin = nullptr;
 };
 bool analysis_can_stream(hx_plan *pl, int spin, int nb);
+int analysis_stream_leadin(StreamSweep &s);
 int analysis_stream_plan(hx_plan *pl, int spin, int nb, int nslab, StreamSweep &s);
 int analysis_stream_start(StreamSweep &s);
 int analysis_stream_slab(StreamSweep &s, int k);
diff --git a/heracles_amd/sht.py b/heracles_amd/sht.py
--- a/heracles_amd/sht.py
+++ b/heracles_amd/sht.py
@@ -39,6 +39,11 @@
             self.close()
         except Exception:
             pass
+
+    def set_leadin_resume(self, on: bool = True, cap_bytes: int | None = None, spin0: bool = False):
+        _lib.check(_lib.load().hx_plan_set_leadin_resume(self._h, (2 if spin0 else 1) if on else 0))
+        if cap_bytes is not None:
+            _lib.check(_lib.load().hx_plan_set_leadin_cap(self._h, int(cap_bytes)))
 
     @property
     def scratch_bytes(self) -> int:
diff --git a/include/hxsht.h b/include/hxsht.h
--- a/include/hxsht.h
+++ b/include/hxsht.h
@@ -37,6 +37,8 @@
 void hx_plan_destroy(hx_plan *plan);
 int64_t hx_plan_scratch_bytes(const hx_plan *plan);
 int hx_plan_release_scratch(hx_plan *plan);
+int hx_plan_set_leadin_resume(hx_plan *plan, int on);
+int hx_plan_set_leadin_cap(hx_plan *plan, int64_t bytes);
 int hx_set_scratch_budget(double bytes);
 int hx_plan_last_chunks(const hx_plan *plan);
 int hx_measure_peaks(double *out4);
```

Result: faster. 436.4 (median of 6 runs) (+1.9%).
